# drdh/Homophily-MARL

Measured on AMD Instinct MI355X. Metric: agent_steps_per_sec, higher is better.
Workload: dtype fp32

## Files before the change

__graft_entry__.py:

```python
import os
import subprocess
import sys

ROOT = os.path.dirname(os.path.abspath(__file__))
if ROOT not in sys.path:
    sys.path.insert(0, ROOT)

CSRC = os.path.join(ROOT, "homophily_marl_amd", "csrc")
HIP_SOURCES = ["ssd_env.hip", "ssd_learner.hip", "ssd_policy.hip", "ssd_policy_mfma.hip", "ssd_gru_seq.hip", "ssd_bmm.hip", "ssd_abi.hip"]
HIP_LIB = os.path.join(ROOT, "homophily_marl_amd", "libssd_hip.so")
HIPCC_FLAGS = ["--offload-arch=gfx950", "-O3", "-std=c++17", "-fPIC", "-shared", "-ffp-contract=off",
               "-fno-fast-math", "-Wall", "-Wno-unused-function", "-mllvm", "-amdgpu-kernarg-preload-count=14"]


def _stale(target, sources):
    if not os.path.exists(target):
        return True
    t = os.path.getmtime(target)
    return any(os.path.getmtime(s) > t for s in sources)


def build(force=False):
    srcs = [os.path.join(CSRC, s) for s in HIP_SOURCES]
    hdrs = [os.path.join(CSRC, h) for h in os.listdir(CSRC) if h.endswith(".h")] + [os.path.join(ROOT, "include", "ssd_hip.h")]
    if force or _stale(HIP_LIB, srcs + hdrs + [os.path.abspath(__file__)]):
        from concurrent.futures import ThreadPoolExecutor
        hipcc = os.environ.get("HIPCC", "/opt/rocm/bin/hipcc")
        objdir = os.path.join(ROOT, "build", "obj")
        os.makedirs(objdir, exist_ok=True)
        flags = [f for f in HIPCC_FLAGS if f != "-shared"]
        jobs = []
        for src in srcs:
            obj = os.path.join(objdir, os.path.basename(src)[:-4] + ".o")
            if force or _stale(obj, [src] + hdrs + [os.path.abspath(__file__)]):
                jobs.append([hipcc] + flags + ["-c", src, "-o", obj])
        for cmd in jobs:
            print("[build]", " ".join(cmd), flush=True)
        with ThreadPoolExecutor(max_workers=min(len(jobs), os.cpu_count() or 1) or 1) as pool:
            rcs = list(pool.map(subprocess.call, jobs))
        if any(rcs):
            raise RuntimeError("hipcc failed (%s)" % rcs)
        objs = [os.path.join(objdir, os.path.basename(src)[:-4] + ".o") for src in srcs]
        cmd = [hipcc, "--offload-arch=gfx950", "-shared", "-fPIC", "-o", HIP_LIB] + objs
        print("[build]", " ".join(cmd), flush=True)
        subprocess.check_call(cmd)
    from oracle import oracle_py
    oracle_py.build(force=force)
    ref_mk = os.path.join(ROOT, "oracle", "build_ref.py")
    if os.path.isdir("/root/reference") and os.path.exists(ref_mk):
        subprocess.check_call([sys.executable, ref_mk])
    import homophily_marl_amd
    from homophily_marl_amd import abi
    abi.load_library()


def smoke():
    import numpy as np
    import torch
    from homophily_marl_amd import abi
    from homophily_marl_amd.envs.native import NativeEnv
    from oracle.oracle_py import OracleEnv

    assert torch.cuda.is_available(), "smoke() needs a GPU"
    kw = dict(map="default5", num_agents=5, n_env=64, view_size=7, episode_limit=100, rng_mode=abi.RNG_COUNTER, seed=7)
    dev = NativeEnv("cleanup", device=0, **kw)
    orc = OracleEnv("cleanup", **kw)
    dev.reset(); orc.reset()
    g = torch.Generator().manual_seed(0)
    for t in range(20):
        acts = torch.randint(0, 9, (64, 5), generator=g, dtype=torch.int32)
        o = dev.step_observe(acts.cuda())
        r = orc.step(acts.numpy())
        assert (o["reward"].cpu().numpy() == r["reward"]).all(), "reward mismatch at step %d" % t
    st, so = dev.export_state(), orc.export_state()
    assert (st["grid"].cpu().numpy() == so["grid"]).all() and (st["pos"].cpu().numpy() == so["pos"]).all()
    assert (o["obs"].cpu().numpy() == orc.observe()["obs"]).all()
    assert dev.poll_error() == 0
    print("smoke ok: 64 envs x 20 steps bit-exact vs oracle; obs", tuple(o["obs"].shape))
    from homophily_marl_amd.run import load_config, setup
    N2, T2 = 32, 12
    cfg = load_config("cleanup", overrides=dict(
        runner="hip_graph", batch_size_run=N2, batch_size=8, buffer_size=N2, buffer_cpu_only=False, store_state=False, obs_storage="code",
        env_args=dict(num_agents=5, map="default5", episode_limit=T2, seed=3), use_cuda=True, save_model=False, runner_stats=False,
        learner_log_interval=10 ** 12))
    torch.manual_seed(0)
    ctx = setup(cfg)
    batch = ctx.runner.run(test_mode=False)
    acts = batch["actions"].squeeze(-1).cpu().numpy().astype(np.int32)
    rew = batch["reward"].cpu().numpy()
    ctx.buffer.insert_episode_batch(batch)
    sample = ctx.buffer.sample(cfg["batch_size"])
    ctx.learner.train(sample[:, :sample.max_t_filled()], ctx.runner.t_env, 0)
    torch.cuda.synchronize()
    assert ctx.runner.env.native.poll_error() == 0
    orc2 = OracleEnv("cleanup", map="default5", num_agents=5, n_env=N2, view_size=7, episode_limit=T2, rng_mode=abi.RNG_COUNTER, seed=3)
    orc2.reset()
    for t in range(T2):
        assert (orc2.step(acts[:, t])["reward"] == rew[:, t]).all(), "stored episode does not replay on the oracle at step %d" % t
    assert all(torch.isfinite(p).all() for p in ctx.mac.parameters())
    print("smoke ok: rollout kernels + learner kernels, %d envs x %d steps stored episode replays on the oracle, one train step" % (N2, T2))


if __name__ == "__main__":
    build(force="--force" in sys.argv)
    if "--smoke" in sys.argv:
        smoke()
```

homophily_marl_amd/abi.py:

```python
import ctypes as C
import os

ABI_VERSION = 10
MAX_AGENTS = 10
MAX_CELLS = 1024
MAX_SITES = 256

ENV_CLEANUP, ENV_HARVEST = 0, 1
RNG_TAPE, RNG_COUNTER = 0, 1
OBS_F32, OBS_BF16, OBS_U8, OBS_CODE = 0, 1, 2, 3
COLOR_SIMPLIFIED, COLOR_FULL = 0, 1
CODE_CLASS, CODE_CHANNEL_MASK = 0, 1
INPUT_LAST_ACTION, INPUT_AGENT_ID, INPUT_REWARD, INPUT_INC_REWARD, INPUT_DISTANCE, INPUT_AGENT_POS = 1, 2, 4, 8, 16, 32
INPUT_OTHERS_LAST_ACTION = 64
INPUT_GATHER_ONEHOT = 0x100
PREV_RECORD_BYTES = 16
INPUT_EXPLICIT = 0x80000000
STREAM_UNIFORM, STREAM_MOVE, STREAM_WASTE, STREAM_SPAWN_ROT = 0, 1, 2, 3

SSD_OK, SSD_ERR_INVALID, SSD_ERR_DEVICE, SSD_ERR_NOMEM, SSD_ERR_UNSUPPORTED = 0, -1, -2, -3, -4
ERRBIT_F16_RANGE = 32
ERR_BAD_RENDER = 64

COPY_BLOCKS_MAX = 32
# ... 217 lines not shown
    return {
        prefix + "abi_version": (C.c_int, []),
        prefix + "last_error": (C.c_char_p, []),
        prefix + "create": (C.c_int, [P(SsdConfig), P(vp)]),
        prefix + "destroy": (C.c_int, [vp]),
        prefix + "reset": (C.c_int, [vp, vp, P(SsdTape), P(SsdStepOut)] + st),
        prefix + "step": (C.c_int, [vp, vp, P(SsdTape), P(SsdStepOut)] + st),
        prefix + "observe": (C.c_int, [vp, P(SsdObsOut)] + st),
        prefix + "export_state": (C.c_int, [vp, P(SsdState)] + st),
        prefix + "import_state": (C.c_int, [vp, P(SsdState)] + st),
        prefix + "get_info": (C.c_int, [vp, P(SsdInfo)]),
        prefix + "build_inputs": (C.c_int, [i32, i32, i32, i32, vp, vp, vp, vp, f32, vp, i32, i32] + st),
        prefix + "incentive_transfer": (C.c_int, [i32, i32, i32, vp, vp, f32, f32, f32, f32,
                                                  vp, vp, vp, vp, vp, vp] + st),
    }


CPU_SIGNATURES = _sigs("ssd_cpu_", False)

vp, i32, i64, u32, u64, f32, P = C.c_void_p, C.c_int32, C.c_int64, C.c_uint32, C.c_uint64, C.c_float, C.POINTER
HIP_SIGNATURES = {name: (C.c_int, args) for name, args in {
    "ssd_step_observe": [vp, vp, P(SsdTape), P(SsdStepOut), P(SsdObsOut), vp],
    "ssd_poll_error": [vp, P(i32)],
    "ssd_set_render": [vp, i32],
    "ssd_render": [vp, vp, i32, vp, vp, i64, vp],
    "ssd_unroll_other": [vp] * 6 + [f32] + [i32] * 4 + [vp] * 3,
    "ssd_column_sums": [vp, vp, i32, i32, i32, vp, vp],
    "ssd_dueling_q_fwd": [vp] * 3 + [i32] * 5 + [vp],
    "ssd_dueling_q_bwd": [vp] * 3 + [i32] * 5 + [vp],
    "ssd_gather_rows": [vp, i32, vp, i32, vp],
    "ssd_sample_ids": [u64, u32, i32, i32, vp, vp],
    "ssd_copy_blocks": [vp, i32, vp],
    "ssd_fill_blocks": [vp, i32, vp],
    "ssd_runner_stats": [vp, vp, vp, i32, i32, vp, vp],
    "ssd_behaviour_stats": [P(SsdBehaviourArgs), vp],
    "ssd_sample_windows": [u64, u32, i32, i32, i32, vp, vp, vp],
    "ssd_gather_windows": [vp, i32, vp, vp, i32, i32, i32, i32, vp],
    "ssd_priority_sample": [P(SsdPrioritySampleArgs), vp],
    "ssd_priority_update": [P(SsdPriorityUpdateArgs), vp],
    "ssd_rollout_priority": [P(SsdRolloutPriorityArgs), vp],
    "ssd_clip_adam_step": [P(SsdClipAdamArgs), vp],
    "ssd_td_sim_loss": [P(SsdTdLossArgs), i32, vp],
    "ssd_encoder": [vp, i32, i32, i32, i32, vp, vp, vp, vp, vp, i32, i32, i32, vp, i64, vp, vp],
    "ssd_conv_leaky": [vp, i32, i32, i32, vp, vp, vp, i32, i32, vp, i64, vp, vp],
    "ssd_store_step_launch": [P(SsdStoreStep), vp],
    "ssd_store_hidden": [P(SsdStoreHiddenArgs), vp],
    "ssd_gru_gates": [vp, vp, vp, i32, i32, vp],
    "ssd_gru_gates_fwd": [vp] * 5 + [i32, i32, vp],
    "ssd_gru_gates_bwd": [vp] * 7 + [i32, i32, vp],
    "ssd_dueling_pick": [vp, i32, i32, vp, vp, vp, u32, i32, i32, i32, vp, vp, u32, vp],
    "ssd_gru_seq_fwd": [vp] * 6 + [i32] * 3 + [vp],
    "ssd_gru_seq_bwd": [vp] * 9 + [i32] * 3 + [vp],
    "ssd_gru_seq_fwd_parts": [vp, i32, vp, vp, i32] + [vp] * 3 + [i32] * 3 + [vp],
    "ssd_gru_seq_bwd_parts": [vp] * 5 + [i32, vp, i32] + [vp] * 3 + [i32] * 4 + [vp],
    "ssd_gru_seq_fwd_h0": [vp, i32, vp, vp, i32, vp, i64, i64] + [vp] * 3 + [i32] * 3 + [vp],
    "ssd_gru_seq_bwd_h0": [vp] * 5 + [i32, vp, i32] + [vp] * 3 + [i32] * 4 + [vp],
    "ssd_bias_bmm_fwd": [vp] * 4 + [i32] * 4 + [vp],
    "ssd_bias_bmm_leaky_fwd": [vp] * 4 + [i32] * 4 + [vp],
    "ssd_bias_bmm_leaky_bwd": [vp] * 8 + [i32] * 4 + [vp],
    "ssd_bias_bmm_bwd": [vp] * 7 + [i32] * 4 + [vp],
    "ssd_bias_bmm2_fwd": [vp] * 5 + [i32] * 7 + [vp],
    "ssd_bias_bmm2_bwd_w": [vp] * 5 + [i32] * 7 + [vp],
    "ssd_bias_bmm_bwd_x": [vp] * 3 + [i32] * 4 + [i64, vp],
    "ssd_dueling_head_fwd": [vp] * 2 + [i32] * 5 + [vp],
    "ssd_dueling_head_bwd": [vp] * 3 + [i32] * 5 + [vp],
    "ssd_bmm_reserve_scratch": [vp],
    "ssd_set_learner_precision": [i32],
    "ssd_learner_precision": [],
    "ssd_conv_wgrad_partial_rows": [i32],
    "ssd_conv_wgrad_codes": [vp, vp, vp, i32, i32, vp],
    "ssd_build_inputs_width": [i32, i32, u32],
    "ssd_build_inputs_flags": [i32, i32, i32, i32, u32, vp, vp, vp, vp, f32, vp, i32, i32, vp],
    "ssd_policy_head_env": [P(SsdPolicyHead), vp],
    "ssd_policy_head_inc": [P(SsdPolicyHead), vp],
    "ssd_policy_head_plan": [i32] * 3 + [P(i32)] * 3,
    "ssd_policy_pack_head": [P(SsdPolicyHeadParams), i32, vp, vp],
    "ssd_policy_encode": [P(SsdPolicyEncodeArgs), vp],
    "ssd_policy_head_inc_encode": [P(SsdPolicyHead), P(SsdPolicyEncodeArgs), vp],
    "ssd_policy_pack_encoder_lut": [vp, vp, vp, i32, i32, vp, vp, vp],
    "ssd_policy_pack_encoder": [vp, vp, vp, i32, i32, vp, vp, vp],
    "ssd_numeric_status": [P(i32)],
}.items()}
HIP_SIGNATURES.update(_sigs("ssd_", True))


def onehot_rows(n_agents, n_actions, flags):
    return 1 + 2 * n_actions + (n_agents * n_actions if flags & INPUT_OTHERS_LAST_ACTION else 0)


def policy_image_bytes(precision):
    return (56 * precision + 8) * 1024


def policy_tail_piece(precision):
    return 56 * precision + 2 * precision


def policy_frag_piece(precision, F, term):
    if F < 8:
        c, ot = F & 1, F >> 1
    elif F < 56:
        G = (F - 8) % 24
        c, ot = (8 if F >= 32 else 2) + 2 * (G >> 3) + (G & 1), (G & 7) >> 1
    else:
        return 56 * precision + 2 * term + (F - 56)
    return 4 * precision * c + 4 * term + ot


def policy_head_plan(n_env, n_agents, fused_with_encoder=False):
    lib = load_library()
    a, b, c = C.c_int32(0), C.c_int32(0), C.c_int32(0)
    check(lib, lib.ssd_policy_head_plan(n_env, n_agents, int(fused_with_encoder), C.byref(a), C.byref(b), C.byref(c)))
    return a.value, b.value, c.value


def encode_edge_supported(V):
    return ENCODE_EDGE_MIN <= V <= ENCODE_EDGE_MAX and V % 2 == 1


def encode_band_rows(V):
    O = V - 2
    nb = 1 if O <= 13 else min(ENCODE_BANDS_MAX, (O + 9) // 10)
    return (O + nb - 1) // nb


def encode_bands(V):
    return (V - 2 + encode_band_rows(V) - 1) // encode_band_rows(V)


def encode_lut_ksteps(V):
    O, R, nb = V - 2, encode_band_rows(V), encode_bands(V)
    return (nb - 1) * ((R * O + 3) // 4) + ((O - (nb - 1) * R) * O + 3) // 4


def encode_frag_bytes(V, precision, layout=ENCODE_LAYOUT_TOEPLITZ):
    if layout == ENCODE_LAYOUT_LUT:
        return ENCODE_LUT_TABLE_BYTES, encode_lut_ksteps(V) * 2 * precision * 1024
    units = 29 * 2 * 3 if V == 31 else 13 * 3
    return precision * 9 * 1024, units * 2 * precision * 1024


def code_agent_stride(V):
    return (V * V + 15) & ~15


def behaviour_len(n, A):
    return 12 * n + n * A + 3 * n * n + 3


def behaviour_layout(n, A):
    blocks = (("reward_sum", (n,)), ("clean_sum", (n,)), ("clean_steps", (n,)), ("harvest_steps", (n,)), ("harvest_time", (n,)),
              ("action_count", (n, A)), ("inc_count", (n, n, 3)), ("recv_on_clean", (n,)), ("recv_on_reward", (n,)), ("role_count", (n, 4)),
              ("cleaners_hist", (n + 1,)), ("n_episodes", (1,)), ("n_steps", (1,)))
    out, off = {}, 0
    for name, shape in blocks:
        out[name] = (off, shape)
        size = 1
        for s in shape:
            size *= s
        off += size
    assert off == behaviour_len(n, A)
    return out


def behaviour_blocks(vec, n, A):
    import numpy as np
    vec = np.asarray(vec, dtype=np.float64).reshape(-1)
    assert vec.size == behaviour_len(n, A), (vec.size, n, A)
    return {k: vec[o:o + int(np.prod(s))].reshape(s).copy() for k, (o, s) in behaviour_layout(n, A).items()}


def behaviour_summary(vec, n, A):
    b = behaviour_blocks(vec, n, A)
    n_ep, n_steps = max(1.0, float(b["n_episodes"][0])), max(1.0, float(b["n_steps"][0]))
    inc, roles = b["inc_count"], b["role_count"].sum(axis=0)
    pairs = max(1, n * (n - 1)) * n_steps
    clean = b["clean_sum"]
    out = {"cleaners_per_env_mean": float((b["cleaners_hist"] * range(n + 1)).sum() / n_ep)}
    for k, name in enumerate(BEHAVIOUR_ROLES):
        out["role_%s_frac" % name] = float(roles[k] / (n * n_ep))
    out["inc_pos_rate"] = float(inc[..., 1].sum() / pairs)
    out["inc_neg_rate"] = float(inc[..., 2].sum() / pairs)
    out["rollout_incentives_to_cleanup_per"] = float(b["recv_on_clean"].sum() / (b["clean_steps"].sum() + 1e-6))
    out["rollout_incentives_to_harvest_per"] = float(b["recv_on_reward"].sum() / (b["reward_sum"].sum() + 1e-6))
    out["rollout_value_give_mean"] = float((inc[..., 1].sum() + inc[..., 2].sum()) / (n * n_steps))
    out["rollout_value_receive_mean"] = float((inc[..., 1].sum() - inc[..., 2].sum()) / (n * n_steps))
    out["harvest_time_mean"] = float(b["harvest_time"].sum() / max(1.0, b["harvest_steps"].sum()))
    out["clean_share_max"] = float(clean.max() / clean.sum()) if clean.sum() > 0 else 0.0
    return out


_PKG_DIR = os.path.dirname(os.path.abspath(__file__))
HIP_LIB_PATH = os.environ.get("SSD_HIP_LIB_PATH", os.path.join(_PKG_DIR, "libssd_hip.so"))
_lib = None


def bind(lib, signatures):
    missing = []
    for name, (res, args) in signatures.items():
        try:
            fn = getattr(lib, name)
        except AttributeError:
            missing.append(name)
            continue
        fn.restype = res
        fn.argtypes = args
    if missing:
        raise ImportError("native library is missing symbols: " + ", ".join(missing))
    return lib


def load_library():
    global _lib
    if _lib is None:
        import torch
        if not os.path.exists(HIP_LIB_PATH):
            raise ImportError(
                "%s not found: build it with `python -c 'import __graft_entry__ as g; g.build()'` "
                "(hipcc --offload-arch=gfx950).  There is no CPU fallback." % HIP_LIB_PATH)
        lib = C.CDLL(HIP_LIB_PATH)
        bind(lib, HIP_SIGNATURES)
        ver = lib.ssd_abi_version()
        if ver != ABI_VERSION:
            raise ImportError("libssd_hip.so ABI version %d != %d" % (ver, ABI_VERSION))
        _lib = lib
    return _lib


class SsdError(RuntimeError):
    pass


def check(lib, rc, err_fn="ssd_last_error"):
    if rc != 0:
        msg = getattr(lib, err_fn)()
        raise SsdError("ssd error %d: %s" % (rc, msg.decode() if msg else "?"))
```

homophily_marl_amd/controllers/homophily_controller.py:

```python
import numpy as np
import torch as th
import torch.nn as nn
import torch.nn.functional as F

from ..components.action_selectors import REGISTRY as action_REGISTRY
from ..modules.agents import REGISTRY as agent_REGISTRY
from .. import ops


class HomophilyMAC(nn.Module):
    def __init__(self, scheme, groups, args):
        super().__init__()
        self.n_agents = args.n_agents
        self.args = args
        self.shipped_flags = bool(args.obs_last_action and args.obs_agent_id and args.obs_reward and args.obs_inc_reward
                                  and args.obs_agent_pos and not getattr(args, "obs_others_last_action", False)
                                  and not getattr(args, "obs_distance", False))
        self.input_flags = None if getattr(args, "obs_others_last_action", False) else (
            1 * bool(args.obs_last_action) | 2 * bool(args.obs_agent_id) | 4 * bool(args.obs_reward) | 8 * bool(args.obs_inc_reward)
            | 16 * bool(getattr(args, "obs_distance", False)) | 32 * bool(args.obs_agent_pos))
        self.input_flags_all = ((self.input_flags if self.input_flags is not None else
                                 (1 * bool(args.obs_last_action) | 2 * bool(args.obs_agent_id) | 4 * bool(args.obs_reward)
                                  | 8 * bool(args.obs_inc_reward) | 16 * bool(getattr(args, "obs_distance", False)) | 32 * bool(args.obs_agent_pos)))
                                | 64 * bool(getattr(args, "obs_others_last_action", False)))
# ... 90 lines not shown
            ops.build_inputs_tail(tail, 0, last_actions, last_reward, last_actions_inc, pos, self.pos_scale, A, t0,
                                  flags=None if self.shipped_flags else self.input_flags_all)
            return th.cat([feat, tail], dim=1)
        dev = feat.device
        if t0:
            last_actions = th.full((B, n), -1, dtype=th.long, device=dev)
            last_reward = th.zeros(B, n, device=dev)
            last_actions_inc = th.zeros(B, n, n, dtype=th.long, device=dev)
        had = (last_actions >= 0).unsqueeze(-1).float()
        onehot = F.one_hot(last_actions.clamp(min=0), A).float() * had
        parts = [feat.reshape(B, n, F0)]
        if a.obs_last_action:
            parts.append(onehot)
        if a.obs_agent_id:
            parts.append(th.eye(n, device=dev).unsqueeze(0).expand(B, -1, -1))
        if a.obs_reward:
            parts.append(th.sign(last_reward.float()).unsqueeze(-1))
        if a.obs_inc_reward:
            m = last_actions_inc * self.inc_mask_actions.squeeze(-1).to(last_actions_inc.dtype)
            recv = (m == 1).sum(dim=1) - (m == 2).sum(dim=1)
            parts.append(th.sign(recv.float()).unsqueeze(-1))
        if getattr(a, "obs_others_last_action", False):
            parts.append(onehot.reshape(B, 1, n * A).expand(-1, n, -1))
        if getattr(a, "obs_distance", False):
            parts.append(1.0 - (pos.unsqueeze(2) - pos.unsqueeze(1)).norm(dim=-1) / self.pos_scale)
        if a.obs_agent_pos:
            parts.append(pos / self.pos_scale)
        return th.cat([x.reshape(B * n, -1).float() for x in parts], dim=1)

    def unroll(self, batch):
        shared = self.unroll_shared(batch)
        parts, wh, bh = self.unroll_pre(batch, shared)
        he, hi = ops.gru_sequence_parts(parts, batch.max_seq_length, batch.batch_size, wh, bh, h0=self.stored_h0(batch))
        return self.agent.unroll_post(he, hi, shared["other"])

    def stored_h0(self, batch):
        if not getattr(self.args, "train_stored_state", False):
            return None
        H = self.args.rnn_hidden_dim
        h = batch["hidden"][:, 0].detach()
        return [h[..., :H].transpose(0, 1), h[..., H:].transpose(0, 1)]

    def unroll_shared(self, batch):
        a = self.args
        B, T, n = batch.batch_size, batch.max_seq_length, self.n_agents
        obs = batch["obs"]
        codes = None
        if obs.dtype == th.uint8:
            if a.rgb_input and self.agent.encoder_kernel_shape and ops.encode_codes_supported(obs):
                codes = obs
            else:
                ops._leaving_kernels("encode_codes", obs, "no encoder kernel for %s windows" % (tuple(obs.shape[-2:]),))
                obs = self.expand_codes(obs)
        acts = batch["actions"].squeeze(-1)
        prev = lambda x, fill: th.cat([th.full_like(x[:, :1], fill), x[:, :-1]], dim=1)
        on_dev = batch["reward"].is_cuda
        kernel_tail = (self.shipped_flags or on_dev) and a.rgb_input and self.input_shape > a.obs_dim_net
        hist = None if (kernel_tail and on_dev) else (
            prev(acts, -1).reshape(B * T, n), prev(batch["reward"], 0).reshape(B * T, n),
            prev(batch["actions_inc"].squeeze(-1), 0).reshape(B * T, n, n), batch["agent_pos"].reshape(B * T, n, 2))
        sh = dict(obs=None if codes is not None else (obs.float() if a.rgb_input else obs), codes=codes, hist=hist, tail=None)
        if on_dev and acts.dtype == th.long:
            sh["onehot"] = None
            sh["other"], sh["act_tm"] = ops.unroll_other(acts, batch["agent_pos"], batch["agent_orientation"], batch["reward"], batch["clean_num"],
                                                         batch["apple_den"], self.pos_scale, a.n_actions)
        else:
            onehot = F.one_hot(acts, num_classes=a.n_actions)
            sh.update(onehot=onehot, act_tm=None,
                      other=self.agent.unroll_other(onehot, batch["agent_pos"] / self.pos_scale, batch["agent_orientation"], batch["reward"],
                                                    batch["clean_num"], batch["apple_den"], th.float32))
        if kernel_tail:
            tail = th.empty(B * T * n, self.input_shape - a.obs_dim_net, dtype=th.float32, device=batch["obs"].device)
            flags = None if self.shipped_flags else self.input_flags_all
            if hist is None:
                ops.build_inputs_tail(tail, 0, acts.reshape(B * T, n), batch["reward"].reshape(B * T, n),
                                      batch["actions_inc"].squeeze(-1).reshape(B * T, n, n), batch["agent_pos"].reshape(B * T, n, 2),
                                      self.pos_scale, a.n_actions, False, flags=flags, seq_len=T)
            else:
                ops.build_inputs_tail(tail, 0, hist[0], hist[1], hist[2], hist[3], self.pos_scale, a.n_actions, False, flags=flags)
            sh["tail"] = tail
        return sh

    def unroll_pre(self, batch, shared):
        a = self.args
        B, T, n = batch.batch_size, batch.max_seq_length, self.n_agents
        obs = shared["obs"]
        if shared.get("codes") is not None:
            feat = self.agent.rgb_preprocess_codes(shared["codes"].reshape(B * T * n, a.obs_dims[0], a.obs_dims[1]))
        elif a.rgb_input:
            feat = self.agent.rgb_preprocess(obs.reshape(B * T * n, 3, a.obs_dims[0], a.obs_dims[1]))
        else:
            feat = obs.reshape(B * T * n, -1)
        if shared["tail"] is not None:
            inputs = th.cat([feat, shared["tail"]], dim=1).reshape(B, T, n, -1)
        else:
            inputs = self.assemble_inputs(feat, *shared["hist"], False).reshape(B, T, n, -1)
        return self.agent.unroll_pre(inputs, shared["onehot"], act_tm=shared.get("act_tm"))

    def _build_inputs(self, batch, t):
        if self.args.rgb_input:
            feat = self.encode_obs(batch["obs"][:, t])
        else:
            feat = batch["obs"][:, t].reshape(batch.batch_size * self.n_agents, -1)
        if t == 0:
            return self.assemble_inputs(feat, None, None, None, batch["agent_pos"][:, t], True)
        return self.assemble_inputs(feat, batch["actions"][:, t - 1].squeeze(-1), batch["reward"][:, t - 1],
                                    batch["actions_inc"][:, t - 1].squeeze(-1), batch["agent_pos"][:, t], False)

    def _get_input_shape(self, scheme):
        a = self.args
        shape = a.obs_dim_net if a.rgb_input else scheme["obs"]["vshape"]
        if a.obs_last_action:
            shape += scheme["actions_onehot"]["vshape"][0]
        if a.obs_agent_id:
            shape += self.n_agents
        shape += int(bool(a.obs_reward)) + int(bool(a.obs_inc_reward))
        if getattr(a, "obs_others_last_action", False):
            shape += scheme["actions_onehot"]["vshape"][0] * self.n_agents
        if getattr(a, "obs_distance", False):
            shape += self.n_agents
        if a.obs_agent_pos:
            shape += 2
        return shape
```

homophily_marl_amd/csrc/ssd_abi.hip:

```cpp
#include <cmath>
#include <cstdio>
#include <cstring>
#include <new>
#include <vector>

#include "ssd_device.h"

using namespace ssd;

struct ssd_env {
    DevSpec hs;
    DevSpec* dspec;
    DevState st;
    int device;
    int n_spawn;
    uint32_t* beam_rec;
    uint8_t* render_lut;
    uint8_t host_lut[64];
};

static thread_local char g_err[512] = "";
static int fail(int code, const char* fmt, const char* a = "") {
    std::snprintf(g_err, sizeof g_err, fmt, a);
    return code;
}
#define HIP_TRY(expr)                                                                   \
    do {                                                                                \
        hipError_t e_ = (expr);                                                         \
        if (e_ != hipSuccess) return fail(SSD_ERR_DEVICE, #expr ": %s", hipGetErrorString(e_)); \
    } while (0)

static uint32_t magic(uint32_t d) { return d <= 1 ? 0xFFFFFFFFu : (uint32_t)(0x100000000ull / d) + 1u; }

extern "C" {

int ssd_abi_version(void) { return SSD_ABI_VERSION; }
const char* ssd_last_error(void) { return g_err; }

static uint32_t draw_threshold(double p) { return p >= 1.0 ? (1u << 24) : !(p > 0.0) ? 0u : (uint32_t)std::ceil(p * 16777216.0); }

int ssd_create(const ssd_config* cfg, ssd_env** out) {
    if (!cfg || !out || !cfg->ascii_map) return fail(SSD_ERR_INVALID, "null argument");
    if (cfg->n_agents < 1 || cfg->n_agents > SSD_MAX_AGENTS) return fail(SSD_ERR_INVALID, "n_agents out of range (1..10)");
    if (cfg->height < 3 || cfg->width < 3 || cfg->height > 255 || cfg->width > 255 || cfg->height * cfg->width > SSD_MAX_CELLS)
        return fail(SSD_ERR_INVALID, "map size out of range");
    if (cfg->n_env < 1) return fail(SSD_ERR_INVALID, "n_env must be >= 1");
    if (cfg->view_size < 0 || cfg->view_size > 31) return fail(SSD_ERR_INVALID, "view_size out of range (0..31)");
    {
        const long V = 2L * cfg->view_size + 1, pm = (cfg->height + 2L * cfg->view_size) * (cfg->width + 2L * cfg->view_size);
        const long per_wave = 2L * ((cfg->height * cfg->width + 15) & ~15) + pm + 16 + cfg->n_agents * 3L * V * V + 32 + 64 + (cfg->n_agents * SSD_CODE_AGENT_STRIDE(V) <= 2560 ? cfg->n_agents : 1) * SSD_CODE_AGENT_STRIDE(V) + 16;
        if (per_wave * 4 > 160 * 1024) return fail(SSD_ERR_INVALID, "map / view_size / n_agents exceed the LDS budget of one workgroup");
    }
    if (cfg->spawn_rotation > 3) return fail(SSD_ERR_INVALID, "spawn_rotation must be -1..3");
    if (cfg->env_kind != SSD_ENV_CLEANUP && cfg->env_kind != SSD_ENV_HARVEST) return fail(SSD_ERR_INVALID, "env_kind");
    if (cfg->rng_mode != SSD_RNG_TAPE && cfg->rng_mode != SSD_RNG_COUNTER) return fail(SSD_ERR_INVALID, "rng_mode");

    ssd_env* E = new (std::nothrow) ssd_env();
    if (!E) return fail(SSD_ERR_NOMEM, "host allocation failed");
    std::memset(E, 0, sizeof *E);
    DevSpec& S = E->hs;
    S.kind = cfg->env_kind; S.H = cfg->height; S.W = cfg->width; S.HW = S.H * S.W; S.GS = (S.HW + 15) & ~15;
    S.n = cfg->n_agents; S.N = cfg->n_env; S.v = cfg->view_size; S.V = 2 * S.v + 1; S.VV = S.V * S.V; S.VVp = (S.VV + 3) & ~3;
    S.Wp = S.W + 2 * S.v; S.PMS = ((S.H + 2 * S.v) * S.Wp + 15) & ~15;
    S.vshift = 0; while ((1 << S.vshift) < S.V) ++S.vshift;
    S.episode_limit = cfg->episode_limit; S.spawn_rotation = cfg->spawn_rotation < 0 ? -1 : cfg->spawn_rotation;
    S.obs_color = cfg->obs_color == SSD_COLOR_FULL ? SSD_COLOR_FULL : SSD_COLOR_SIMPLIFIED;
    S.rng_mode = cfg->rng_mode; S.n_actions = S.kind == SSD_ENV_CLEANUP ? 9 : 8;
    S.env_id_base = cfg->env_id_base; S.seed_lo = (uint32_t)cfg->seed; S.seed_hi = (uint32_t)(cfg->seed >> 32);
    S.magic_W = magic(S.W); S.magic_V = magic(S.V); S.magic_VV = magic(S.VV); S.magic_3VV = magic(3 * S.VV); S.magic_HW = magic(S.HW);
    S.thr_dep = cfg->threshold_depletion; S.thr_res = cfg->threshold_restoration;
    S.p_waste = cfg->waste_spawn_prob; S.p_apple = cfg->apple_respawn_prob;
    for (int i = 0; i < 4; ++i) { S.harvest_p[i] = cfg->harvest_spawn_prob[i]; S.harvest_thr[i] = draw_threshold(S.harvest_p[i]); }
    if ((long)S.n * 3 * S.VV >= 65536) { delete E; return fail(SSD_ERR_INVALID, "n_agents * 3 * V * V must stay below 65536"); }
    if ((long)lds_per_wave(S) * kWavesPerBlock > 160 * 1024) { delete E; return fail(SSD_ERR_INVALID, "k_env's LDS slices exceed the 160 KiB of a workgroup"); }
    if (code_gather_end(S, kCodeGroupMax) > lds_planes_bytes(S)) { delete E; return fail(SSD_ERR_INVALID, "class-code gather overruns its LDS planes"); }

    std::vector<int> spawn;
    for (int i = 0; i < S.HW; ++i) {
        const char ch = cfg->ascii_map[i];
        uint8_t code = C_EMPTY;
        bool overflow = false;
        if (ch == '@') code = C_WALL;
        else if (ch == 'P') spawn.push_back(i);
        else if (S.kind == SSD_ENV_CLEANUP) {
            if (ch == 'B') { if (S.n_apple < SSD_MAX_SITES) S.apple[S.n_apple++] = (uint16_t)i; else overflow = true; }
            else if (ch == 'H') { code = C_WASTE; if (S.n_waste < SSD_MAX_SITES) S.waste[S.n_waste++] = (uint16_t)i; else overflow = true; }
            else if (ch == 'R') code = C_RIVER;
            else if (ch == 'S') code = C_STREAM;
        } else if (ch == 'A') { code = C_APPLE; if (S.n_apple < SSD_MAX_SITES) S.apple[S.n_apple++] = (uint16_t)i; else overflow = true; }
// ... 680 lines not shown
                       (long)h0_row_stride);
    return launched();
}

int ssd_gru_seq_bwd(const float* dhs, const float* hs, const float* rzn, const float* ghn, const float* wh, float* d_gi, float* dgh,
                    float* d_wh, float* d_bh_part, int32_t T, int32_t G, int32_t B, void* stream) {
    if (int rc = gru_seq_bwd_check("ssd_gru_seq_bwd", 0, &dhs, hs, rzn, ghn, &wh, 1, &d_gi, 0, dgh, d_wh, d_bh_part, T, G, G, B)) return rc;
    launch_gru_seq_bwd(&dhs, hs, rzn, ghn, &wh, 1, &d_gi, 0, dgh, d_wh, d_bh_part, T, G, G, B, (hipStream_t)stream);
    return launched();
}
int ssd_gru_seq_bwd_parts(const float* const* dhs_parts, const float* hs, const float* rzn, const float* ghn, const float* const* wh_parts, int32_t n_wparts,
                          float* const* d_gi_parts, int32_t n_parts, float* dgh, float* d_wh, float* d_bh_part, int32_t T, int32_t G, int32_t G_grad, int32_t B,
                          void* stream) {
    if (int rc = gru_seq_bwd_check("ssd_gru_seq_bwd_parts", 1, dhs_parts, hs, rzn, ghn, wh_parts, n_wparts, d_gi_parts, n_parts, dgh, d_wh, d_bh_part, T, G, G_grad, B))
        return rc;
    launch_gru_seq_bwd(dhs_parts, hs, rzn, ghn, wh_parts, n_wparts, d_gi_parts, n_parts, dgh, d_wh, d_bh_part, T, G, G_grad, B, (hipStream_t)stream);
    return launched();
}
int ssd_gru_seq_bwd_h0(const float* const* dhs_parts, const float* hs, const float* rzn, const float* ghn, const float* const* wh_parts, int32_t n_wparts,
                       float* const* d_gi_parts, int32_t n_parts, float* dgh, float* d_wh, float* d_bh_part, int32_t T, int32_t G, int32_t G_grad, int32_t B,
                       void* stream) {
    if (int rc = gru_seq_bwd_check("ssd_gru_seq_bwd_h0", 0, dhs_parts, hs, rzn, ghn, wh_parts, n_wparts, d_gi_parts, n_parts, dgh, d_wh, d_bh_part, T, G, G_grad, B))
        return rc;
    launch_gru_seq_bwd(dhs_parts, hs, rzn, ghn, wh_parts, n_wparts, d_gi_parts, n_parts, dgh, d_wh, d_bh_part, T, G, G_grad, B, (hipStream_t)stream, true);
    return launched();
}

int ssd_bias_bmm_fwd(const float* x, const float* w, const float* b, float* y, int32_t n, int32_t rows, int32_t in, int32_t out, void* stream) {
    if (!x || !w || !b || !y || n < 1 || rows < 1 || in < 1 || out < 1) return fail(SSD_ERR_INVALID, "bad argument");
    if (launch_bias_bmm_fwd(x, w, b, y, n, rows, in, out, (hipStream_t)stream)) return fail(SSD_ERR_UNSUPPORTED, "ssd_bias_bmm_fwd: a weight / operand set of 2^30 elements or more");
    return launched();
}
int ssd_bias_bmm_leaky_fwd(const float* x, const float* w, const float* b, float* y, int32_t n, int32_t rows, int32_t in, int32_t out, void* stream) {
    if (!x || !w || !b || !y || n < 1 || rows < 1 || in < 1 || out < 1) return fail(SSD_ERR_INVALID, "bad argument");
    if (launch_bias_bmm_fwd(x, w, b, y, n, rows, in, out, (hipStream_t)stream, 1)) return fail(SSD_ERR_UNSUPPORTED, "ssd_bias_bmm_leaky_fwd: a weight / operand set of 2^30 elements or more");
    return launched();
}
int ssd_bias_bmm_leaky_bwd(const float* g, const float* y, const float* x, const float* w, float* dx, float* dw, float* db, const float* slope_of,
                           int32_t n, int32_t rows, int32_t in, int32_t out, void* stream) {
    if (!g || !y || n < 1 || rows < 1 || in < 1 || out < 1) return fail(SSD_ERR_INVALID, "bad argument");
    if ((dx && !w) || ((dw || db) && !x) || (slope_of && !dx)) return fail(SSD_ERR_INVALID, "dx needs w, dw / db need x, slope_of needs dx");
    if (launch_bias_bmm_bwd(g, x, w, dx, dw, db, slope_of, n, rows, in, out, (hipStream_t)stream, 0, 0, y)) return fail(SSD_ERR_UNSUPPORTED, "ssd_bias_bmm_leaky_bwd: an operand set of 2^30 elements or more");
    return launched();
}
int ssd_bias_bmm_bwd(const float* g, const float* x, const float* w, float* dx, float* dw, float* db, const float* slope_of, int32_t n,
                     int32_t rows, int32_t in, int32_t out, void* stream) {
    if (!g || n < 1 || rows < 1 || in < 1 || out < 1) return fail(SSD_ERR_INVALID, "bad argument");
    if ((dx && !w) || ((dw || db) && !x) || (slope_of && !dx)) return fail(SSD_ERR_INVALID, "dx needs w, dw / db need x, slope_of needs dx");
    if (launch_bias_bmm_bwd(g, x, w, dx, dw, db, slope_of, n, rows, in, out, (hipStream_t)stream)) return fail(SSD_ERR_UNSUPPORTED, "ssd_bias_bmm_bwd: an operand set of 2^30 elements or more");
    return launched();
}

int ssd_dueling_head_fwd(const float* y, float* q, int32_t n, int32_t T, int32_t B, int32_t inner, int32_t K, void* stream) {
    if (!y || !q || n < 1 || T < 1 || B < 1 || inner < 1 || K < 1 || K > 15) return fail(SSD_ERR_INVALID, "bad argument");
    launch_dueling_q(y, y + K, q, nullptr, nullptr, nullptr, n, T, B, inner, K, (hipStream_t)stream, K + 1, 1, nullptr);
    return launched();
}
int ssd_dueling_head_bwd(const float* dq, float* dy, float* gs, int32_t n, int32_t T, int32_t B, int32_t inner, int32_t K, void* stream) {
    if (!dq || !dy || n < 1 || T < 1 || B < 1 || inner < 1 || K < 1 || K > 15) return fail(SSD_ERR_INVALID, "bad argument");
    launch_dueling_q(nullptr, nullptr, nullptr, dq, dy, dy + K, n, T, B, inner, K, (hipStream_t)stream, K + 1, 1, gs);
    return launched();
}
int ssd_bias_bmm2_fwd(const float* x1, const float* x2, const float* w, const float* b, float* y, int32_t n, int32_t rows, int32_t in1, int32_t in2,
                      int32_t out, int32_t x1_div, int32_t x2_shared, void* stream) {
    if (!x1 || !x2 || !w || !b || !y || n < 1 || rows < 1 || in1 < 1 || in2 < 1 || out < 1) return fail(SSD_ERR_INVALID, "bad argument");
    const int rc = launch_bias_bmm2_fwd(x1, x2, w, b, y, n, rows, in1, in2, out, x1_div, x2_shared, (hipStream_t)stream);
    if (rc == -3) return fail(SSD_ERR_INVALID, "ssd_bias_bmm2_fwd: in1 a multiple of 16, rows a multiple of x1_div >= 1");
    if (rc) return fail(SSD_ERR_UNSUPPORTED, "ssd_bias_bmm2_fwd: a weight / operand set of 2^30 elements or more");
    return launched();
}
int ssd_bias_bmm2_bwd_w(const float* g, const float* x1, const float* x2, float* dw, float* db, int32_t n, int32_t rows, int32_t in1, int32_t in2,
                        int32_t out, int32_t x1_div, int32_t x2_shared, void* stream) {
    if (!g || !x1 || !x2 || (!dw && !db) || n < 1 || rows < 1 || in1 < 1 || in2 < 1 || out < 1) return fail(SSD_ERR_INVALID, "bad argument");
    const int rc = launch_bias_bmm_bwd(g, x1, nullptr, nullptr, dw, db, nullptr, n, rows, in1 + in2, out, (hipStream_t)stream, 0, 0, nullptr, x2, in1, x1_div,
                                       x2_shared, 0);
    if (rc == -3) return fail(SSD_ERR_INVALID, "ssd_bias_bmm2_bwd_w: in1 a multiple of 16, rows a multiple of x1_div >= 1");
    if (rc) return fail(SSD_ERR_UNSUPPORTED, "ssd_bias_bmm2_bwd_w: an operand set of 2^30 elements or more");
    return launched();
}
int ssd_bias_bmm_bwd_x(const float* g, const float* w, float* dx, int32_t n, int32_t rows, int32_t in, int32_t out, int64_t w_set, void* stream) {
    if (!g || !w || !dx || n < 1 || rows < 1 || in < 1 || out < 1 || w_set < (int64_t)in * out) return fail(SSD_ERR_INVALID, "bad argument");
    if (launch_bias_bmm_bwd(g, nullptr, w, dx, nullptr, nullptr, nullptr, n, rows, in, out, (hipStream_t)stream, 0, 0, nullptr, nullptr, 0, 1, 0, (long)w_set))
        return fail(SSD_ERR_UNSUPPORTED, "ssd_bias_bmm_bwd_x: an operand set of 2^30 elements or more");
    return launched();
}
int ssd_bmm_reserve_scratch(void* stream) {
    if (!bmm_scratch((hipStream_t)stream)) return fail(SSD_ERR_DEVICE, "ssd_bmm_reserve_scratch: allocation failed (inside a stream capture?)");
    return SSD_OK;
}
int ssd_set_learner_precision(int32_t precision) {
    if (precision != 1 && precision != 2) return fail(SSD_ERR_INVALID, "ssd_set_learner_precision: 1 (bf16) or 2 (f32)");
    set_learner_precision(precision);
    return SSD_OK;
}
int ssd_learner_precision(void) { return learner_precision(); }
int ssd_conv_wgrad_partial_rows(int32_t rows) { return rows < 1 ? 0 : conv_wgrad_partial_rows(rows); }
static bool encode_edge_ok(int V) { return V >= SSD_ENCODE_EDGE_MIN && V <= SSD_ENCODE_EDGE_MAX && (V & 1); }
#define SSD_EDGE_MSG ": view_edge must be odd, 3 .. 63 (view_size 1 .. 31)"

int ssd_conv_wgrad_codes(const uint8_t* codes, const float* d_conv, float* partial, int32_t rows, int32_t view_edge, void* stream) {
    if (!codes || !d_conv || !partial || rows < 1) return fail(SSD_ERR_INVALID, "bad argument");
    if (!encode_edge_ok(view_edge)) return fail(SSD_ERR_UNSUPPORTED, "ssd_conv_wgrad_codes" SSD_EDGE_MSG);
    if (launch_conv_wgrad(codes, d_conv, partial, rows, view_edge, (hipStream_t)stream)) return fail(SSD_ERR_UNSUPPORTED, "ssd_conv_wgrad_codes" SSD_EDGE_MSG);
    return launched();
}

static int check_encode(const ssd_policy_encode_args* a) {
    if (!a || !a->codes || !a->conv_frags || !a->lin_frags || !a->conv_b || !a->lin_b || a->rows < 1 || a->n_agents < 1 || a->rows % a->n_agents)
        return fail(SSD_ERR_INVALID, "bad argument");
    if (!encode_edge_ok(a->view_edge)) return fail(SSD_ERR_UNSUPPORTED, "ssd_policy_encode" SSD_EDGE_MSG "; use ssd_conv_leaky + GEMM");
    const bool shipped = a->view_edge == 15 || a->view_edge == 31;
    if (!shipped && a->layout != SSD_ENCODE_LAYOUT_LUT)
        return fail(SSD_ERR_UNSUPPORTED, "ssd_policy_encode: the Toeplitz layout is instantiated for 15 x 15 / 31 x 31 windows; other edges take SSD_ENCODE_LAYOUT_LUT");
    if (a->precision != 0 && a->precision != 1 && a->precision != 2) return fail(SSD_ERR_INVALID, "precision must be 1 (bf16) or 2 (f32-equivalent)");
    if (a->alphabet != SSD_CODE_CLASS && a->alphabet != SSD_CODE_CHANNEL_MASK) return fail(SSD_ERR_INVALID, "alphabet");
    if (a->layout != SSD_ENCODE_LAYOUT_TOEPLITZ && a->layout != SSD_ENCODE_LAYOUT_LUT) return fail(SSD_ERR_INVALID, "layout");
    if (a->act && shipped && a->layout != SSD_ENCODE_LAYOUT_TOEPLITZ)
        return fail(SSD_ERR_INVALID, "the activation output (training forward) takes the Toeplitz images at 15 x 15 / 31 x 31");
    const int bands = SSD_ENCODE_BANDS(a->view_edge);
    if (bands == 1 ? (!a->out || a->part || a->out_stride < 32) : (!a->part || a->out)) return fail(SSD_ERR_INVALID, "one band writes `out`, several bands write `part`");
    if ((reinterpret_cast<uintptr_t>(a->conv_frags) | reinterpret_cast<uintptr_t>(a->lin_frags) | reinterpret_cast<uintptr_t>(a->part)) & 15)
        return fail(SSD_ERR_INVALID, "conv_frags / lin_frags / part must be 16-byte aligned");
    const long VV = (long)a->view_edge * a->view_edge;
    if (a->agent_stride < VV || a->env_stride < (long)a->n_agents * a->agent_stride || a->slot_stride < 0 || (a->slot_stride && !a->slot_t))
        return fail(SSD_ERR_INVALID, "env_stride / slot_stride / agent_stride / slot_t");
    if (a->code_bytes < (long)(a->rows / a->n_agents - 1) * a->env_stride + (long)(a->n_agents - 1) * a->agent_stride + VV)
        return fail(SSD_ERR_INVALID, "code_bytes does not cover the rows");
    if (a->slot_t_copy && (!a->slot_t || a->slot_t_copy == a->slot_t)) return fail(SSD_ERR_INVALID, "slot_t_copy needs a distinct slot_t");
    if (a->slot_add < 0 || (a->slot_add && !a->slot_t)) return fail(SSD_ERR_INVALID, "slot_add needs slot_t");
    return SSD_OK;
}

int ssd_policy_encode(const ssd_policy_encode_args* a, void* stream) {
    if (const int bad = check_encode(a)) return bad;
    const int rc = launch_policy_encode(a, (hipStream_t)stream);
    if (rc) return fail(SSD_ERR_DEVICE, "hipFuncSetAttribute(max dynamic LDS) failed");
    return launched();
}

int ssd_policy_pack_encoder_lut(const float* conv_w, const float* conv_b, const float* lin_w, int32_t view_edge, int32_t precision, void* table,
                                void* lin_frags, void* stream) {
    if (!conv_w || !conv_b || !lin_w || !table || !lin_frags) return fail(SSD_ERR_INVALID, "null argument");
    if (precision != 1 && precision != 2) return fail(SSD_ERR_INVALID, "precision must be 1 or 2");
    if ((reinterpret_cast<uintptr_t>(table) | reinterpret_cast<uintptr_t>(lin_frags)) & 15) return fail(SSD_ERR_INVALID, "images must be 16-byte aligned");
    if (!encode_edge_ok(view_edge)) return fail(SSD_ERR_UNSUPPORTED, "ssd_policy_pack_encoder_lut" SSD_EDGE_MSG);
    if (launch_pack_encoder_lut(conv_w, conv_b, lin_w, view_edge, precision, table, lin_frags, (hipStream_t)stream))
        return fail(SSD_ERR_UNSUPPORTED, "ssd_policy_pack_encoder_lut" SSD_EDGE_MSG);
    return launched();
}

int ssd_policy_pack_encoder(const float* conv_w, const float* conv_b, const float* lin_w, int32_t view_edge, int32_t precision, void* conv_frags,
                            void* lin_frags, void* stream) {
    if (!conv_w || !conv_b || !lin_w || !conv_frags || !lin_frags) return fail(SSD_ERR_INVALID, "null argument");
    if (precision != 1 && precision != 2) return fail(SSD_ERR_INVALID, "precision must be 1 or 2");
    if ((reinterpret_cast<uintptr_t>(conv_frags) | reinterpret_cast<uintptr_t>(lin_frags)) & 15) return fail(SSD_ERR_INVALID, "fragment images must be 16-byte aligned");
    if (launch_pack_encoder(conv_w, conv_b, lin_w, view_edge, precision, conv_frags, lin_frags, (hipStream_t)stream))
        return fail(SSD_ERR_UNSUPPORTED, "ssd_policy_pack_encoder: view_edge must be 15 or 31");
    return launched();
}

int ssd_policy_pack_head(const ssd_policy_head_params* p, int32_t precision, void* image, void* stream) {
    if (!p || !image || !p->fc1_w || !p->fc1_b || !p->fc2_w || !p->fc2_b || !p->fc2_v_w || !p->fc2_v_b) return fail(SSD_ERR_INVALID, "null argument");
    for (int g = 0; g < 3; ++g) if (!p->w_i[g] || !p->w_h[g] || !p->b_i[g] || !p->b_h[g]) return fail(SSD_ERR_INVALID, "null GRU parameter");
    if (precision != 1 && precision != 2) return fail(SSD_ERR_INVALID, "precision must be 1 or 2");
    if (p->input_flags & SSD_INPUT_GATHER_ONEHOT) {
        const uint32_t fl = p->input_flags;
// ... 154 lines not shown
```

homophily_marl_amd/csrc/ssd_bmm.hip:

```cpp
#include <hip/hip_runtime.h>
#include <mutex>
#include <stdint.h>
#include "../../include/ssd_hip.h"

namespace ssd {

using f32x4 = __attribute__((ext_vector_type(4))) float;
typedef float f32x4_u __attribute__((ext_vector_type(4), aligned(4)));

struct BmmK {
    const float *x, *w, *b, *g;
    float *y, *dx, *dw, *db;
    const float* slope_of;
    int n, R, I, O;
    long x_set, g_set;
    const float* act_y;
    int leaky;
    const float* x2; int I1, x1_div; long x2_set;
    uint32_t x1_magic;
    long w_set;
    float* part;
    int row_chunks;
};
constexpr int BMM_PART = 272;

__device__ __forceinline__ float ld32(const float* base, uint32_t idx) {
    return *reinterpret_cast<const float*>(reinterpret_cast<const uint8_t*>(base) + (size_t)(idx * 4u));
}
__device__ __forceinline__ f32x4 mfma4(float a, float b, f32x4 c) { return __builtin_amdgcn_mfma_f32_16x16x4f32(a, b, c, 0, 0, 0); }
using bf8 = __attribute__((ext_vector_type(8))) __bf16;
__device__ __forceinline__ f32x4 mfma32b(const float (&a)[8], const float (&b)[8], f32x4 c) {
    bf8 x, y;
#pragma unroll
    for (int j = 0; j < 8; ++j) { x[j] = (__bf16)a[j]; y[j] = (__bf16)b[j]; }
    return __builtin_amdgcn_mfma_f32_16x16x32_bf16(x, y, c, 0, 0, 0);
}
static int g_learner_precision = 2;
int learner_precision() { return g_learner_precision; }
void set_learner_precision(int p) { g_learner_precision = p == 1 ? 1 : 2; }

__device__ __forceinline__ f32x4 load4(const float* p, int k0, int len) {
    if (k0 + 4 <= len) return *reinterpret_cast<const f32x4_u*>(p + k0);
    f32x4 v = {0.f, 0.f, 0.f, 0.f};
#pragma unroll
    for (int r = 0; r < 4; ++r)
        if (k0 + r < len) v[r] = p[k0 + r];
    return v;
}

constexpr int BMM_TPW = 3;
template <bool XV, bool BF = false>
__global__ __launch_bounds__(256) void k_bias_bmm_fwd(BmmK a) {
    const int lane = threadIdx.x & 63, wave = __builtin_amdgcn_readfirstlane(threadIdx.x >> 6);
    const int m = lane & 15, q = lane >> 4;
    const int R = a.R, I = a.I, O = a.O;
    const int otiles = (O + 15) >> 4, groups = (otiles + BMM_TPW - 1) / BMM_TPW, rtiles = (R + 15) >> 4;
    const int unit = blockIdx.x * 4 + wave;
    if (unit >= rtiles * groups) return;
    const int g = blockIdx.y, row0 = (unit / groups) * 16, t0 = (unit % groups) * BMM_TPW;
    const int rowc = row0 + m < R ? row0 + m : R - 1;
    const bool two = a.x2 != nullptr;
    const int I1 = two ? a.I1 : I;
    const float* xs = a.x + (two ? (size_t)g * (size_t)(R / a.x1_div) * I1 : (size_t)g * R * I);
    const uint32_t xrow = two ? (uint32_t)(rowc / a.x1_div) * (uint32_t)I1 : (uint32_t)rowc * (uint32_t)I;
    const float* x2s = two ? a.x2 + (size_t)g * a.x2_set : a.x;
    const uint32_t x2row = (uint32_t)rowc * (uint32_t)(I - I1);
    const float* wg = a.w + (size_t)g * (a.w_set ? a.w_set : (long)I * O);
    f32x4 acc[BMM_TPW];
#pragma unroll
    for (int t = 0; t < BMM_TPW; ++t) {
        const int o = 16 * (t0 + t) + m;
        const float bv = (t0 + t < otiles && o < O) ? a.b[(size_t)g * O + o] : 0.f;
        acc[t] = f32x4{bv, bv, bv, bv};
    }
    const int chunks = (I + 15) >> 4;
    int oc[BMM_TPW]; bool on[BMM_TPW];
#pragma unroll
    for (int t = 0; t < BMM_TPW; ++t) {
        const int o = 16 * (t0 + t) + m;
        on[t] = t0 + t < otiles && o < O; oc[t] = on[t] ? o : 0;
    }
    struct Chunk { float x[4]; float w[BMM_TPW][4]; };
    auto fetch = [&](int c, Chunk& d) {
        const int k0 = 16 * c + 4 * q;
        if constexpr (XV) {
            const int kc = k0 < I ? k0 : I - 4;
            const bool second = 16 * c >= I1;
            const float* base = second ? x2s : xs;
            const uint32_t off = second ? x2row + (uint32_t)(kc - I1) : xrow + (uint32_t)kc;
            const f32x4 v = *reinterpret_cast<const f32x4_u*>(reinterpret_cast<const uint8_t*>(base) + (size_t)(off * 4u));
#pragma unroll
            for (int r = 0; r < 4; ++r) d.x[r] = v[r];
        }
#pragma unroll
        for (int r = 0; r < 4; ++r) {
            const int k = k0 + r < I ? k0 + r : I - 1;
            if constexpr (!XV) {
                const bool sec = k >= I1;
                d.x[r] = ld32(sec ? x2s : xs, sec ? x2row + (uint32_t)(k - I1) : xrow + (uint32_t)k);
            }
#pragma unroll
            for (int t = 0; t < BMM_TPW; ++t) d.w[t][r] = ld32(wg, (uint32_t)k * (uint32_t)O + (uint32_t)oc[t]);
        }
    };
    auto use = [&](int c, const Chunk& d) {
        const int k0 = 16 * c + 4 * q;
#pragma unroll
        for (int r = 0; r < 4; ++r) {
            const bool kon = k0 + r < I;
            const float xv = kon ? d.x[r] : 0.f;
#pragma unroll
            for (int t = 0; t < BMM_TPW; ++t)
                if (t0 + t < otiles) acc[t] = mfma4(xv, (kon && on[t]) ? d.w[t][r] : 0.f, acc[t]);
        }
    };
    auto use_pair = [&](int c, const Chunk& d0, const Chunk& d1, bool two) {
        const int k0 = 16 * c + 4 * q;
        float xv[8];
#pragma unroll
        for (int r = 0; r < 4; ++r) { xv[r] = k0 + r < I ? d0.x[r] : 0.f; xv[4 + r] = (two && k0 + 16 + r < I) ? d1.x[r] : 0.f; }
#pragma unroll
        for (int t = 0; t < BMM_TPW; ++t) {
            if (t0 + t >= otiles) continue;
            float wv[8];
#pragma unroll
            for (int r = 0; r < 4; ++r) { wv[r] = (k0 + r < I && on[t]) ? d0.w[t][r] : 0.f; wv[4 + r] = (two && k0 + 16 + r < I && on[t]) ? d1.w[t][r] : 0.f; }
            acc[t] = mfma32b(xv, wv, acc[t]);
        }
    };
    Chunk ca, cb;
    fetch(0, ca);
    for (int c = 0; c < chunks; c += 2) {
        if (c + 1 < chunks) fetch(c + 1, cb);
        if constexpr (BF) {
            Chunk cur = ca;
            if (c + 2 < chunks) fetch(c + 2, ca);
            use_pair(c, cur, cb, c + 1 < chunks);
        } else {
            use(c, ca);
            if (c + 1 < chunks) {
                if (c + 2 < chunks) fetch(c + 2, ca);
                use(c + 1, cb);
            }
        }
    }
#pragma unroll
    for (int t = 0; t < BMM_TPW; ++t) {
        const int o = 16 * (t0 + t) + m;
        if (t0 + t >= otiles || o >= O) continue;
#pragma unroll
        for (int r = 0; r < 4; ++r) {
            const int row = row0 + 4 * q + r;
            const float v = acc[t][r];
            if (row < R) a.y[((size_t)g * R + row) * O + o] = (a.leaky && !(v > 0.f)) ? 0.01f * v : v;
        }
    }
}

__device__ __forceinline__ int gridDim_tiles(const BmmK& a) { return ((a.I + 15) >> 4) * ((a.O + 15) >> 4); }
__global__ __launch_bounds__(64) void k_bmm_dw_reduce(BmmK a) {
    const int lane = threadIdx.x, m = lane & 15, q = lane >> 4, tile = blockIdx.x, g = blockIdx.y, C = a.row_chunks;
    const int otiles = (a.O + 15) >> 4, it = tile / otiles, ot = tile - it * otiles, o = 16 * ot + m;
    const float* P = a.part + ((size_t)((size_t)g * gridDim.x + tile) * C) * BMM_PART;
    f32x4 sum = *reinterpret_cast<const f32x4*>(P + 4 * lane);
    float sb = q == 0 ? P[256 + m] : 0.f;
    for (int c = 1; c < C; ++c) {
        sum += *reinterpret_cast<const f32x4*>(P + (size_t)c * BMM_PART + 4 * lane);
        if (q == 0) sb += P[(size_t)c * BMM_PART + 256 + m];
    }
    if (o >= a.O) return;
    if (a.dw) {
#pragma unroll
        for (int r = 0; r < 4; ++r) {
            const int ii = 16 * it + 4 * q + r;
            if (ii < a.I) a.dw[((size_t)g * a.I + ii) * a.O + o] = sum[r];
        }
    }
    if (a.db && it == 0 && q == 0) a.db[(size_t)g * a.O + o] = sb;
}
constexpr int BMM_BWD_WAVES = 16;
template <bool OV, bool ACT, bool BF = false>
__global__ __launch_bounds__(BMM_BWD_WAVES * 64) void k_bias_bmm_bwd(BmmK a, int dw_blocks) {
    __shared__ f32x4 red[BMM_BWD_WAVES][64];
    __shared__ float redb[BMM_BWD_WAVES][16];
    const int lane = threadIdx.x & 63, wave = __builtin_amdgcn_readfirstlane(threadIdx.x >> 6);
    const int m = lane & 15, q = lane >> 4;
    const int g = blockIdx.y;
    const int R = a.R, I = a.I, O = a.O;
    const int itiles = (I + 15) >> 4, otiles = (O + 15) >> 4;
    const float* gg = a.g + (size_t)g * a.g_set;
    if ((int)blockIdx.x >= dw_blocks) {
        const int unit = (blockIdx.x - dw_blocks) * BMM_BWD_WAVES + wave, rtiles = (R + 15) >> 4;
        if (unit >= rtiles * itiles) return;
        const int row0 = (unit / itiles) * 16, i = 16 * (unit % itiles) + m;
        const int rowc = row0 + m < R ? row0 + m : R - 1;
        const float* ws = a.w + (size_t)g * (a.w_set ? a.w_set : (long)I * O);
        const uint32_t grow = (uint32_t)rowc * (uint32_t)O, wrow = (uint32_t)(i < I ? i : I - 1) * (uint32_t)O;
        f32x4 acc = {0.f, 0.f, 0.f, 0.f};
        const int chunks = (O + 15) >> 4;
        struct Pair { f32x4 g, w, y; };
        const float* yy = ACT ? a.act_y + (size_t)g * a.g_set : nullptr;
        auto fetch = [&](int c, Pair& d) {
            const int k0 = 16 * c + 4 * q;
            if constexpr (OV) {
                const uint32_t kb = (uint32_t)(k0 < O ? k0 : O - 4);
                d.g = *reinterpret_cast<const f32x4_u*>(reinterpret_cast<const uint8_t*>(gg) + (size_t)((grow + kb) * 4u));
                d.w = *reinterpret_cast<const f32x4_u*>(reinterpret_cast<const uint8_t*>(ws) + (size_t)((wrow + kb) * 4u));
                if constexpr (ACT) d.y = *reinterpret_cast<const f32x4_u*>(reinterpret_cast<const uint8_t*>(yy) + (size_t)((grow + kb) * 4u));
            } else {
#pragma unroll
                for (int r = 0; r < 4; ++r) {
                    const uint32_t k = (uint32_t)(k0 + r < O ? k0 + r : O - 1);
                    d.g[r] = ld32(gg, grow + k); d.w[r] = ld32(ws, wrow + k);
                    if constexpr (ACT) d.y[r] = ld32(yy, grow + k);
                }
            }
        };
        auto use = [&](int c, const Pair& d) {
            const int k0 = 16 * c + 4 * q;
#pragma unroll
            for (int r = 0; r < 4; ++r) {
                const bool on = k0 + r < O;
                float gv = on ? d.g[r] : 0.f;
                if constexpr (ACT) gv = d.y[r] > 0.f ? gv : 0.01f * gv;
                acc = mfma4(gv, on ? d.w[r] : 0.f, acc);
            }
        };
        auto use_pair = [&](int c, const Pair& d0, const Pair& d1, bool two) {
            const int k0 = 16 * c + 4 * q;
            float gv[8], wv[8];
#pragma unroll
            for (int r = 0; r < 4; ++r) {
                const bool on0 = k0 + r < O, on1 = two && k0 + 16 + r < O;
                float g0 = on0 ? d0.g[r] : 0.f, g1 = on1 ? d1.g[r] : 0.f;
                if constexpr (ACT) { g0 = d0.y[r] > 0.f ? g0 : 0.01f * g0; g1 = (on1 && !(d1.y[r] > 0.f)) ? 0.01f * g1 : g1; }
                gv[r] = g0; gv[4 + r] = g1; wv[r] = on0 ? d0.w[r] : 0.f; wv[4 + r] = on1 ? d1.w[r] : 0.f;
            }
// ... 91 lines not shown
        if (C > 1) {
            float* P = a.part + ((size_t)((size_t)g * gridDim_tiles(a) + tile) * C + chunk) * BMM_PART;
            *reinterpret_cast<f32x4*>(P + 4 * lane) = sum;
            if (q == 0) {
                float sb = redb[0][m];
#pragma unroll
                for (int v = 1; v < BMM_BWD_WAVES; ++v) sb += redb[v][m];
                P[256 + m] = sb;
            }
            return;
        }
        if (a.dw && oon) {
#pragma unroll
            for (int r = 0; r < 4; ++r) {
                const int ii = 16 * it + 4 * q + r;
                if (ii < I) a.dw[((size_t)g * I + ii) * O + o] = sum[r];
            }
        }
        if (a.db && it == 0 && q == 0 && oon) {
            float sb = redb[0][m];
#pragma unroll
            for (int v = 1; v < BMM_BWD_WAVES; ++v) sb += redb[v][m];
            a.db[(size_t)g * O + o] = sb;
        }
    }
}

constexpr size_t BMM_SCRATCH_BYTES = 1 << 20;
constexpr int BMM_SCRATCH_SLOTS = 64;
float* bmm_scratch(hipStream_t stream) {
    struct Slot { hipStream_t stream; float* buf; };
    static Slot slots[64][BMM_SCRATCH_SLOTS] = {};
    static int used[64] = {};
    static std::mutex mu;
    int dev = 0;
    if (hipGetDevice(&dev) != hipSuccess || dev < 0 || dev >= 64) return nullptr;
    std::lock_guard<std::mutex> lock(mu);
    for (int i = 0; i < used[dev]; ++i)
        if (slots[dev][i].stream == stream) return slots[dev][i].buf;
    if (used[dev] == BMM_SCRATCH_SLOTS) return nullptr;
    float* p = nullptr;
    if (hipMalloc((void**)&p, BMM_SCRATCH_BYTES) != hipSuccess) { (void)hipGetLastError(); return nullptr; }
    slots[dev][used[dev]++] = Slot{stream, p};
    return p;
}

int launch_bias_bmm_fwd(const float* x, const float* w, const float* b, float* y, int n, int R, int I, int O, hipStream_t s, int leaky) {
    BmmK k = {};
    k.x = x; k.w = w; k.b = b; k.y = y; k.n = n; k.R = R; k.I = I; k.O = O; k.leaky = leaky;
    const int otiles = (O + 15) / 16, units = ((R + 15) / 16) * ((otiles + BMM_TPW - 1) / BMM_TPW);
    if ((long)I * O >= (1L << 30) || (long)R * I >= (1L << 30)) return -2;
    const dim3 grid((units + 3) / 4, n);
    if (g_learner_precision == 1) {
        if ((I & 3) == 0) hipLaunchKernelGGL((k_bias_bmm_fwd<true, true>), grid, dim3(256), 0, s, k);
        else hipLaunchKernelGGL((k_bias_bmm_fwd<false, true>), grid, dim3(256), 0, s, k);
    } else {
        if ((I & 3) == 0) hipLaunchKernelGGL((k_bias_bmm_fwd<true, false>), grid, dim3(256), 0, s, k);
        else hipLaunchKernelGGL((k_bias_bmm_fwd<false, false>), grid, dim3(256), 0, s, k);
    }
    return 0;
}

int launch_bias_bmm2_fwd(const float* x1, const float* x2, const float* w, const float* b, float* y, int n, int R, int I1, int I2, int O, int x1_div,
                         int x2_shared, hipStream_t s) {
    BmmK k = {};
    const int I = I1 + I2;
    k.x = x1; k.x2 = x2; k.I1 = I1; k.x1_div = x1_div; k.x2_set = x2_shared ? 0 : (long)R * I2;
    k.w = w; k.b = b; k.y = y; k.n = n; k.R = R; k.I = I; k.O = O;
    if ((I1 & 15) || x1_div < 1 || R % x1_div) return -3;
    if ((long)I * O >= (1L << 30) || (long)R * I >= (1L << 30)) return -2;
    const int otiles = (O + 15) / 16, units = ((R + 15) / 16) * ((otiles + BMM_TPW - 1) / BMM_TPW);
    const dim3 grid((units + 3) / 4, n);
    const bool xv = (I2 & 3) == 0;
    if (g_learner_precision == 1) {
        if (xv) hipLaunchKernelGGL((k_bias_bmm_fwd<true, true>), grid, dim3(256), 0, s, k);
        else hipLaunchKernelGGL((k_bias_bmm_fwd<false, true>), grid, dim3(256), 0, s, k);
    } else {
        if (xv) hipLaunchKernelGGL((k_bias_bmm_fwd<true, false>), grid, dim3(256), 0, s, k);
        else hipLaunchKernelGGL((k_bias_bmm_fwd<false, false>), grid, dim3(256), 0, s, k);
    }
    return 0;
}

int launch_bias_bmm_bwd(const float* g, const float* x, const float* w, float* dx, float* dw, float* db, const float* slope_of, int n, int R,
                        int I, int O, hipStream_t s, long x_set, long g_set, const float* act_y, const float* x2, int I1, int x1_div, int x2_shared,
                        long w_set) {
    BmmK k = {};
    k.act_y = act_y;
    if ((long)R * I >= (1L << 30) || (long)R * O >= (1L << 30) || (long)I * O >= (1L << 30)) return -2;
    if (x2) {
        if (dx || (I1 & 15) || x1_div < 1 || R % x1_div) return -3;
        k.x2 = x2; k.I1 = I1; k.x1_div = x1_div; k.x2_set = x2_shared ? 0 : (long)R * (I - I1);
        k.x1_magic = x1_div == 1 ? 0u : (uint32_t)(((1ull << 32) + (uint64_t)x1_div - 1) / (uint64_t)x1_div);
        if (R >= (1 << 28) || (uint64_t)R * (uint64_t)x1_div > (1ull << 32)) return -2;
    }
    k.w_set = w_set;
    k.g = g; k.x = x; k.w = w; k.dx = dx; k.dw = dw; k.db = db; k.slope_of = slope_of; k.n = n; k.R = R; k.I = I; k.O = O;
    k.x_set = x_set ? x_set : (long)R * I; k.g_set = g_set ? g_set : (long)R * O;
    const int dxb = dx ? (((R + 15) / 16) * ((I + 15) / 16) + BMM_BWD_WAVES - 1) / BMM_BWD_WAVES : 0;
    int dwb = (dw || db) ? ((I + 15) / 16) * ((O + 15) / 16) : 0;
    if (dxb + dwb == 0) return 0;
    k.row_chunks = 1;
    const int tiles = dwb;
    if (dwb && (R + 3) / 4 >= 64 * BMM_BWD_WAVES && dwb * n <= 128) {
        int c = 256 / (dwb * n);
        if (c > 8) c = 8;
        float* part = bmm_scratch(s);
        if (c > 1 && part && (size_t)n * dwb * c * BMM_PART * sizeof(float) <= BMM_SCRATCH_BYTES) { k.row_chunks = c; k.part = part; dwb *= c; }
    }
    const dim3 grid(dwb + dxb, n), block(BMM_BWD_WAVES * 64);
    const bool ov = (O & 3) == 0, bf = g_learner_precision == 1;
#define SSD_BWD(OV_, ACT_, BF_) hipLaunchKernelGGL((k_bias_bmm_bwd<OV_, ACT_, BF_>), grid, block, 0, s, k, dwb)
    if (act_y) {
        if (ov) { if (bf) SSD_BWD(true, true, true); else SSD_BWD(true, true, false); }
        else { if (bf) SSD_BWD(false, true, true); else SSD_BWD(false, true, false); }
    } else {
        if (ov) { if (bf) SSD_BWD(true, false, true); else SSD_BWD(true, false, false); }
        else { if (bf) SSD_BWD(false, false, true); else SSD_BWD(false, false, false); }
    }
#undef SSD_BWD
    if (k.row_chunks > 1) hipLaunchKernelGGL(k_bmm_dw_reduce, dim3(tiles, n), dim3(64), 0, s, k);
    return 0;
}


constexpr int CW_ROWS = 4, CW_OUT = 6 * 27 + 6;
template <int CTRL, int ROW_MASK>
__device__ __forceinline__ float dpp_add(float v) {
    return v + __builtin_bit_cast(float, __builtin_amdgcn_update_dpp(0, __builtin_bit_cast(int, v), CTRL, ROW_MASK, 0xF, false));
}
__device__ __forceinline__ float wave_sum_to_lane63(float v) {
    v = dpp_add<0xB1, 0xF>(v);
    v = dpp_add<0x4E, 0xF>(v);
    v = dpp_add<0x124, 0xF>(v);
    v = dpp_add<0x128, 0xF>(v);
    v = dpp_add<0x142, 0xA>(v);
    v = dpp_add<0x143, 0xC>(v);
    return v;
}
template <int V>
__global__ __launch_bounds__(256) void k_conv_wgrad(const uint8_t* __restrict__ codes, const float* __restrict__ d_conv, float* __restrict__ partial, int R) {
    constexpr int O = V - 2, P = O * O, VV = V * V, VVP = (VV + 15) & ~15;
    __shared__ uint8_t win[4][VVP];
    const int lane = threadIdx.x & 63, wave = __builtin_amdgcn_readfirstlane(threadIdx.x >> 6);
    const int wg = blockIdx.x * 4 + wave;
    float acc[6][27], accb[6];
#pragma unroll
    for (int oc = 0; oc < 6; ++oc) {
        accb[oc] = 0.f;
#pragma unroll
        for (int k = 0; k < 27; ++k) acc[oc][k] = 0.f;
    }
    constexpr int PASSES = (P + 63) / 64;
    const int row_begin = wg * CW_ROWS, rows_here = row_begin >= R ? 0 : (R - row_begin < CW_ROWS ? R - row_begin : CW_ROWS);
    const int items = rows_here * PASSES;
    auto fetch = [&](int it, float (&v)[6]) {
        const int row = row_begin + it / PASSES, p = (it % PASSES) * 64 + lane;
        const float* dr = d_conv + (size_t)row * 6 * P;
#pragma unroll
        for (int oc = 0; oc < 6; ++oc) v[oc] = p < P ? dr[oc * P + p] : 0.f;
    };
    float cur[6], nxt[6];
    if (items > 0) fetch(0, nxt);
    for (int it = 0; it < items; ++it) {
#pragma unroll
        for (int oc = 0; oc < 6; ++oc) cur[oc] = nxt[oc];
// ... 123 lines not shown
```

homophily_marl_amd/csrc/ssd_device.h:

```cpp
#pragma once
#include <hip/hip_runtime.h>
#include <stdint.h>

#include "../../include/ssd_hip.h"

namespace ssd {

constexpr int kWave = 64;
#ifndef SSD_WAVES_PER_BLOCK
#define SSD_WAVES_PER_BLOCK 4
#endif
constexpr int kWavesPerBlock = SSD_WAVES_PER_BLOCK;
constexpr int kBlock = kWave * kWavesPerBlock;

enum : int { C_EMPTY = 0, C_WALL = 1, C_APPLE = 2, C_WASTE = 3, C_RIVER = 4, C_STREAM = 5 };
enum : int { O_LEFT = 0, O_RIGHT = 1, O_UP = 2, O_DOWN = 3 };
enum : int { MODE_RESET = 0, MODE_STEP = 1, MODE_STEP_OBS = 2, MODE_OBS = 3 };

struct DevHead {
    int32_t kind, H, W, HW, GS;
    int32_t n, N, V, v, VV, VVp;
    int32_t Wp, PMS;
    int32_t vshift;
    int32_t episode_limit, spawn_rotation, obs_color, rng_mode, n_actions;
// ... 30 lines not shown
    uint8_t* grid;
    uint2* agents;
    EnvHdr* hdr;
    int32_t* err;
    unsigned long long* stamps;
};

struct DevTape {
    const uint8_t* move_order;
    const double* uniforms;
    int32_t ustride;
    const uint8_t* waste_order;
    const uint8_t* spawn_rot;
    const uint8_t* spawn_order;
};

struct DevStepOut {
    float *reward, *clean_num, *apple_den;
    uint8_t* terminated;
    float *collective, *equality;
    int32_t* n_draws;
};

struct DevObsOut {
    void* obs;
    int32_t fmt;
    float *state, *pos, *orient;
    long env_stride, slot_stride;
    int32_t t_slots;
    uint8_t* code;
    int32_t code_agent_stride;
    unsigned long long* stamps;
};

enum : int { ERR_BAD_ACTION = 1, ERR_BAD_TAPE = 2, ERR_KEYERROR = 4, ERR_TAPE_OVERRUN = 8, ERR_SLOT_OVERRUN = 16, ERR_F16_RANGE = 32, ERR_BAD_RENDER = 64 };
int32_t* numeric_err_word();
constexpr float F16_MAX = 65504.f;

__host__ __device__ inline int lds_planes_bytes(const DevHead& s) { return ((s.n * 3 * s.VV + 16) + 15) & ~15; }
__host__ __device__ inline int code_dump_byte(int delta, int n, int VV) { return delta + n * VV; }
__host__ __device__ inline int code_gather_end(const DevHead& s, int ag) {
    return code_dump_byte(15, s.n, s.VV) + ((ag < s.n ? ag : s.n) - 1) * s.VV + 1;
}
constexpr int kCodeGroupMax = 5;
__host__ __device__ inline bool lds_code_all(const DevHead& s) { return s.n * SSD_CODE_AGENT_STRIDE(s.V) <= 2560; }
__host__ __device__ inline int lds_code_bytes(const DevHead& s) { return (lds_code_all(s) ? s.n : 1) * SSD_CODE_AGENT_STRIDE(s.V) + 16; }
#if defined(SSD_STAMPS) && SSD_STAMPS == 2
constexpr int kStampLds = 256;
#else
constexpr int kStampLds = 0;
#endif
__host__ __device__ inline int lds_per_wave(const DevHead& s) {
    int obs = s.PMS + lds_planes_bytes(s);
    if (obs < 512) obs = 512;
    return ((2 * s.GS + obs + 64 + lds_code_bytes(s) + 255) & ~255) + kStampLds;
}

void launch_env(int mode, const DevSpec* spec, const DevSpec& host_spec, DevState st, const int32_t* actions,
                const uint8_t* env_mask, DevTape tape, DevStepOut so, DevObsOut oo, hipStream_t stream, uint32_t* beam_rec = nullptr);
void launch_beam_clear(uint32_t* beam_rec, const uint8_t* env_mask, int n_env, int n_agents, hipStream_t stream);
void launch_render(const DevSpec* spec, const DevSpec& hs, DevState st, const uint32_t* beam_rec, const uint8_t* lut, const int32_t* env_ids,
                   int n_sel, uint8_t* frames, const int32_t* slot, long long slot_stride, hipStream_t stream);

void launch_export(const DevSpec* spec, const DevSpec& hs, DevState st, ssd_state dst, hipStream_t stream);
void launch_import(const DevSpec* spec, const DevSpec& hs, DevState st, ssd_state src, hipStream_t stream);

void launch_build_inputs(int32_t batch, int32_t n, int32_t A, int32_t t0, const int64_t* last_actions,
                         const float* last_reward, const int64_t* last_actions_inc, const float* pos, float pos_scale,
                         float* out, int32_t out_stride, int32_t out_offset, hipStream_t stream);
struct BuildInputsLayout { int o_act, o_id, o_r, o_i, o_oth, o_dist, o_pos, width; };
BuildInputsLayout build_inputs_layout(int n, int A, uint32_t input_flags);
void launch_build_inputs_flags(int32_t batch, int32_t n, int32_t A, int32_t t0, uint32_t input_flags, const int64_t* last_actions,
                               const float* last_reward, const int64_t* last_actions_inc, const float* pos, float pos_scale,
                               float* out, int32_t out_stride, int32_t out_offset, hipStream_t stream);
void launch_incentive_transfer(int32_t B, int32_t T, int32_t n, const int64_t* a_inc, const float* rewards,
                               float effect_ratio, float cost_ratio, float incentive, float seq_len, float* give,
                               float* recv_pos, float* recv_neg, float* recv_zero, float* r_env, float* r_inc,
                               hipStream_t stream);

void launch_column_sums(const float* x, float* out, int G, int R, int C, float* workspace, hipStream_t stream);
void launch_copy_blocks(const ssd_block_copy* blocks, int count, hipStream_t stream);
void launch_clip_adam(const ssd_clip_adam_args* a, hipStream_t stream);
void launch_dueling_q(const float* a, const float* v, float* q, const float* dq, float* da, float* dv, int n, int T, int B, int inner, int K, hipStream_t stream,
                      int ld = 0, int merged = 0, float* gs = nullptr);
void launch_gather_rows(const ssd_row_gather* fields, int count, const int64_t* ids, int n_ids, hipStream_t stream);
void launch_td_sim_loss(const ssd_td_loss_args* a, int mode, hipStream_t stream);
constexpr long long kDefaultLdsLimit = 64 * 1024;
constexpr int kEncoderRowsPerWave = 1, kEncoderRowsPerBlock = 4 * kEncoderRowsPerWave;
constexpr long long encoder_lds_bytes(long long V) { return kEncoderRowsPerBlock * (3 * V * V + 4) * (long long)sizeof(float); }
constexpr long long conv_leaky_lds_bytes(long long V) { return (3 * V * V + 6 * 27 + 6) * (long long)sizeof(float); }
void launch_encoder(const float* obs, int rows, int V, const float* cw, const float* cb, const float* lw, const float* lb, float* out,
                    int out_stride, int n_agents, int agent_major, float* store, long store_env_stride, const int64_t* store_t,
                    hipStream_t s);
void launch_conv_leaky(const float* obs, int rows, int V, const float* cw, const float* cb, float* out, int n_agents, int agent_major,
                       float* store, long store_env_stride, const int64_t* store_t, hipStream_t s);
void launch_store_step(const ssd_store_step* a, hipStream_t s);
void launch_store_hidden(const ssd_store_hidden_args* a, hipStream_t s);
void launch_gru_gates(const float* gi, const float* gh, float* h, int R, int H, hipStream_t s);
void launch_gru_fwd_train(const float* gi, const float* gh, const float* h, float* h_new, float* rzn, int R, int H, hipStream_t s);
void launch_gru_bwd(const float* dh, const float* rzn, const float* gh, const float* h, float* d_gi, float* d_gh, float* dh_prev, int R,
                    int H, hipStream_t s);
int launch_policy_encode(const ssd_policy_encode_args* p, hipStream_t s);
int launch_pack_encoder_lut(const float* cw, const float* cb, const float* lw, int V, int prec, void* table, void* lin_frags, hipStream_t s);
int launch_pack_encoder(const float* cw, const float* cb, const float* lw, int V, int prec, void* conv_frags, void* lin_frags, hipStream_t s);
void launch_pack_head(const ssd_policy_head_params* p, int prec, void* image, hipStream_t s);
void launch_gru_seq_fwd(const float* const* gi_parts, int n_parts, const float* const* wh_parts, const float* const* bh_parts, int n_wparts, float* hs,
                        float* rzn, float* ghn, int T, int G, int B, hipStream_t s, const float* const* h0_parts = nullptr, long h0_set_stride = 0,
                        long h0_row_stride = 0);
void launch_gru_seq_bwd(const float* const* dhs_parts, const float* hs, const float* rzn, const float* ghn, const float* const* wh_parts, int n_wparts,
                        float* const* d_gi_parts, int n_parts, float* dgh, float* d_wh, float* d_bh_part, int T, int G, int Gn, int B, hipStream_t s,
                        bool h0 = false);
int launch_policy_head(const ssd_policy_head* p, int inc, hipStream_t s);
void policy_head_plan(int n_env, int n_agents, int mode, int* wg_per_agent, int* waves_out, int* tiles_per_wave);
int launch_policy_inc_encode(const ssd_policy_head* ph, const ssd_policy_encode_args* pe, hipStream_t s);
int launch_policy_inc_encode_gather(const ssd_policy_head* ph, const ssd_policy_encode_args* pe, hipStream_t s);
int conv_wgrad_partial_rows(int R);
int launch_conv_wgrad(const uint8_t* codes, const float* d_conv, float* partial, int R, int V, hipStream_t s);
void launch_unroll_other(const int64_t* actions, const float* pos, const float* orient, const float* reward, const float* clean, const float* den,
                         float pos_scale, int B, int T, int n, int A, float* other, float* act_tm, hipStream_t stream);
float* bmm_scratch(hipStream_t stream);
int learner_precision();
void set_learner_precision(int p);
void launch_fill_blocks(const ssd_block_fill* blocks, int count, hipStream_t stream);
void launch_runner_stats(const float* coll, const float* eq, const float* ret, int n_env, int n_ret, double* acc, hipStream_t stream);
void launch_behaviour_stats(const ssd_behaviour_args* a, hipStream_t stream);
void launch_sample_draw(uint64_t seed, uint32_t call, int population, int count, int n_starts, int64_t* ids, int64_t* t0, hipStream_t stream);
void launch_gather_windows(const ssd_window_field* fields, int count, const int64_t* ids, const int64_t* t0, int n_ids, int src_slots,
                           int win_slots, int burn_in, hipStream_t stream);
void launch_priority_sample(const ssd_priority_sample_args* a, hipStream_t stream);
void launch_priority_update(const ssd_priority_update_args* a, hipStream_t stream);
void launch_rollout_priority(const ssd_rollout_priority_args* a, hipStream_t stream);
int launch_bias_bmm_fwd(const float* x, const float* w, const float* b, float* y, int n, int R, int I, int O, hipStream_t s, int leaky = 0);
int launch_bias_bmm_bwd(const float* g, const float* x, const float* w, float* dx, float* dw, float* db, const float* slope_of, int n, int R,
                        int I, int O, hipStream_t s, long x_set = 0, long g_set = 0, const float* act_y = nullptr, const float* x2 = nullptr, int I1 = 0,
                        int x1_div = 1, int x2_shared = 0, long w_set = 0);
int launch_bias_bmm2_fwd(const float* x1, const float* x2, const float* w, const float* b, float* y, int n, int R, int I1, int I2, int O, int x1_div,
                         int x2_shared, hipStream_t s);
#ifdef SSD_STAMPS
void set_policy_stamps(unsigned long long* buf);
#endif
void launch_dueling_pick(const float* av, int R, int A, const uint8_t* avail, const float* eps, const int64_t* step, uint32_t seed,
                         int n_agents, int B, int pairs, int64_t* actions, float* q_out, uint32_t env_id_base, hipStream_t s);

}
```

homophily_marl_amd/csrc/ssd_learner.hip:

```cpp
#include "ssd_device.h"

namespace ssd {

__global__ void k_build_inputs(int32_t rows, int32_t n, int32_t A, int32_t t0, const int64_t* __restrict__ last_actions,
                               const float* __restrict__ last_reward, const int64_t* __restrict__ last_actions_inc,
                               const float* __restrict__ pos, float pos_scale, float* __restrict__ out,
                               int32_t out_stride, int32_t out_offset) {
    const int width = A + n + 4;
    const size_t total = (size_t)rows * width;
    for (size_t idx = (size_t)blockIdx.x * blockDim.x + threadIdx.x; idx < total; idx += (size_t)gridDim.x * blockDim.x) {
        const int row = (int)(idx / width), k = (int)(idx - (size_t)row * width);
        const int b = row / n, i = row - b * n;
        const int agent_major = t0 & 2;
        const int hist_T = t0 >> 8;
        const int t_zero = (t0 & 1) || (hist_T && b % hist_T == 0);
        const size_t pb = hist_T ? (size_t)b - 1 : (size_t)b, prow = pb * n + i;
        float v;
        if (k < A) v = (!t_zero && last_actions[prow] == k) ? 1.f : 0.f;
        else if (k < A + n) v = (k - A == i) ? 1.f : 0.f;
        else if (k == A + n) {
            const float r = t_zero ? 0.f : last_reward[prow];
            v = (float)((r > 0.f) - (r < 0.f));
        } else if (k == A + n + 1) {
            int recv = 0;
// ... 500 lines not shown
__global__ __launch_bounds__(64 * BEH_WAVES) void k_behaviour_partials(const int64_t* __restrict__ actions, const int64_t* __restrict__ actions_inc,
                                                                       const float* __restrict__ reward, const float* __restrict__ clean,
                                                                       int n_env, int T, int n, int A, long long* __restrict__ ws) {
    __shared__ long long cnt[BEH_LEN_MAX];
    const int len = SSD_BEHAVIOUR_LEN(n, A);
    for (int k = threadIdx.x; k < len; k += 64 * BEH_WAVES) cnt[k] = 0;
    __syncthreads();
    const int lane = threadIdx.x & 63, wave = threadIdx.x >> 6;
    const int tpw = 64 / n, nn = n * n;
    const int tl = lane / n, j = lane - tl * n;
    const bool active = tl < tpw;
    const int o_act = 5 * n, o_inc = o_act + n * A, o_rc = o_inc + 3 * nn, o_role = o_rc + 2 * n, o_hist = o_role + 4 * n, o_ep = o_hist + n + 1;
    long long s_r = 0, s_c = 0, s_cl = 0, s_hv = 0, s_ht = 0, s_rc = 0, s_rr = 0, envs = 0;
    const size_t row = (size_t)(T + 1) * n;
    for (long b = (long)blockIdx.x * BEH_WAVES + wave; b < n_env; b += (long)gridDim.x * BEH_WAVES) {
        const int64_t* a_e = actions + (size_t)b * row;
        const int64_t* ai_e = actions_inc + (size_t)b * row * n;
        const float* r_e = reward + (size_t)b * row;
        const float* c_e = clean + (size_t)b * row;
        int C = 0, Hh = 0;
        for (int t0 = 0; t0 < T; t0 += tpw) {
            const int t = t0 + tl;
            const bool valid = active && t < T;
            const int tc = valid ? t : 0, m = tc * n + j;
            long long v[SSD_MAX_AGENTS];
#pragma unroll
            for (int i = 0; i < SSD_MAX_AGENTS; ++i) v[i] = ai_e[tc * nn + (i < n ? i : j) * n + j];
            const long long a = a_e[m];
            const int r = valid ? beh_round(r_e[m]) : 0, c = valid ? beh_round(c_e[m]) : 0;
            int rv = 0;
#pragma unroll
            for (int i = 0; i < SSD_MAX_AGENTS; ++i) {
                const bool ok = valid && i < n && i != j;
                if (ok && (unsigned long long)v[i] < 3ull) beh_add(cnt, o_inc + (i * n + j) * 3 + (int)v[i], 1);
                rv += (ok && v[i] == 1) - (ok && v[i] == 2);
            }
            if (valid && (unsigned long long)a < (unsigned long long)A) beh_add(cnt, o_act + j * A + (int)a, 1);
            const int cl = c > 0, hv = r > 0;
            s_r += r; s_c += c; s_cl += cl; s_hv += hv; s_ht += hv ? t : 0;
            s_rc += cl ? rv : 0; s_rr += (long long)r * rv;
            C += cl; Hh += hv;
        }
        int Cs = 0, Hs = 0;
        for (int k = 0; k < tpw; ++k) {
            const int src = (lane + k * n) & 63;
            Cs += __shfl(C, src); Hs += __shfl(Hh, src);
        }
        const bool agent = lane < n, cleaner = agent && Cs > Hs;
        if (agent) beh_add(cnt, o_role + lane * 4 + ((Cs == 0 && Hs == 0) ? 0 : Cs > Hs ? 1 : Hs > Cs ? 2 : 3), 1);
        const int n_cleaners = __popcll(__ballot(cleaner));
        if (lane == 0) beh_add(cnt, o_hist + n_cleaners, 1);
        envs += 1;
    }
    if (active) {
        beh_add(cnt, j, s_r); beh_add(cnt, n + j, s_c); beh_add(cnt, 2 * n + j, s_cl); beh_add(cnt, 3 * n + j, s_hv); beh_add(cnt, 4 * n + j, s_ht);
        beh_add(cnt, o_rc + j, s_rc); beh_add(cnt, o_rc + n + j, s_rr);
    }
    if (lane == 0) { beh_add(cnt, o_ep, envs); beh_add(cnt, o_ep + 1, envs * T); }
    __syncthreads();
    for (int k = threadIdx.x; k < len; k += 64 * BEH_WAVES) ws[(size_t)blockIdx.x * len + k] = cnt[k];
}

__global__ __launch_bounds__(256) void k_behaviour_finish(const long long* __restrict__ ws, int groups, int len, double* __restrict__ acc) {
    for (int k = threadIdx.x; k < len; k += 256) {
        long long s = 0;
        for (int g = 0; g < groups; ++g) s += ws[(size_t)g * len + k];
        acc[k] += (double)s;
    }
}

void launch_behaviour_stats(const ssd_behaviour_args* a, hipStream_t stream) {
    int groups = a->n_env / BEH_WAVES + (a->n_env % BEH_WAVES ? 1 : 0);
    if (groups > SSD_BEHAVIOUR_MAX_GROUPS) groups = SSD_BEHAVIOUR_MAX_GROUPS;
    long long* ws = reinterpret_cast<long long*>(a->workspace);
    hipLaunchKernelGGL(k_behaviour_partials, dim3(groups), dim3(64 * BEH_WAVES), 0, stream, a->actions, a->actions_inc, a->reward, a->clean_num,
                       a->n_env, a->t_slots - 1, a->n_agents, a->n_actions, ws);
    hipLaunchKernelGGL(k_behaviour_finish, dim3(1), dim3(256), 0, stream, ws, groups, SSD_BEHAVIOUR_LEN(a->n_agents, a->n_actions), a->acc);
}

static int grid_for(size_t total);
template <bool BWD>
__global__ __launch_bounds__(256) void k_dueling_q(const float* __restrict__ a, const float* __restrict__ v, float* __restrict__ q,
                                                   const float* __restrict__ dq, float* __restrict__ da, float* __restrict__ dv, int n, int T, int B,
                                                   int inner, int K, int ld, int merged, float* __restrict__ gs) {
    const long rows = (long)T * B * inner, total = rows * n;
    const int vld = merged ? ld : 1;
    for (long idx = (long)blockIdx.x * 256 + threadIdx.x; idx < total; idx += (long)gridDim.x * 256) {
        const int i = (int)(idx / rows);
        const long r = idx - (long)i * rows;
        const long tb = r / inner;
        const int j = (int)(r - tb * inner), t = (int)(tb / B), b = (int)(tb - (long)t * B);
        const size_t qo = ((((size_t)b * T + t) * n + i) * inner + j) * K, ao = ((size_t)i * rows + r) * ld;
        float x[16], sum = 0.f;
        for (int k = 0; k < K; ++k) { x[k] = BWD ? dq[qo + k] : a[ao + k]; sum += x[k]; }
        if (BWD) {
            const float mean = sum / (float)K;
            for (int k = 0; k < K; ++k) da[ao + k] = x[k] - mean;
            dv[((size_t)i * rows + r) * vld] = sum;
            if (gs && j == 0) {
                float g[17];
                for (int k = 0; k <= K; ++k) g[k] = 0.f;
                for (int jj = 0; jj < inner; ++jj) {
                    const size_t qj = qo + (size_t)jj * K;
                    float y[16], s2 = 0.f;
                    for (int k = 0; k < K; ++k) { y[k] = dq[qj + k]; s2 += y[k]; }
                    const float m2 = s2 / (float)K;
                    for (int k = 0; k < K; ++k) g[k] += y[k] - m2;
                    g[K] += s2;
                }
                float* go = gs + ((size_t)i * (rows / inner) + tb) * (K + 1);
                for (int k = 0; k <= K; ++k) go[k] = g[k];
            }
        } else {
            const float vv = v[((size_t)i * rows + r) * vld], mean = sum / (float)K;
            for (int k = 0; k < K; ++k) q[qo + k] = (vv + x[k]) - mean;
        }
    }
}

void launch_dueling_q(const float* a, const float* v, float* q, const float* dq, float* da, float* dv, int n, int T, int B, int inner, int K,
                      hipStream_t stream, int ld, int merged, float* gs) {
    const size_t total = (size_t)n * T * B * inner;
    if (ld <= 0) ld = K;
    if (dq) hipLaunchKernelGGL(k_dueling_q<true>, dim3(grid_for(total)), dim3(256), 0, stream, a, v, q, dq, da, dv, n, T, B, inner, K, ld, merged, gs);
    else hipLaunchKernelGGL(k_dueling_q<false>, dim3(grid_for(total)), dim3(256), 0, stream, a, v, q, dq, da, dv, n, T, B, inner, K, ld, merged, gs);
}

struct GatherTable { ssd_row_gather f[SSD_COPY_BLOCKS_MAX]; };
typedef uint32_t u32_unaligned __attribute__((aligned(1)));
__global__ __launch_bounds__(256) void k_gather_rows(GatherTable t, const int64_t* __restrict__ ids) {
    const ssd_row_gather f = t.f[blockIdx.y];
    const uint8_t* src = static_cast<const uint8_t*>(f.src) + (size_t)ids[blockIdx.z] * f.row_bytes;
    uint8_t* dst = static_cast<uint8_t*>(f.dst) + (size_t)blockIdx.z * f.row_bytes;
    const long words = f.row_bytes >> 2;
    for (long i = (long)blockIdx.x * 256 + threadIdx.x; i < words; i += (long)gridDim.x * 256)
        *reinterpret_cast<u32_unaligned*>(dst + 4 * i) = *reinterpret_cast<const u32_unaligned*>(src + 4 * i);
    if (blockIdx.x == 0 && (long)threadIdx.x < (f.row_bytes & 3)) dst[4 * words + threadIdx.x] = src[4 * words + threadIdx.x];
}

void launch_gather_rows(const ssd_row_gather* fields, int count, const int64_t* ids, int n_ids, hipStream_t stream) {
    GatherTable t;
    int64_t most = 4;
    for (int i = 0; i < SSD_COPY_BLOCKS_MAX; ++i) {
        t.f[i] = fields[i < count ? i : 0];
        if (i < count && fields[i].row_bytes > most) most = fields[i].row_bytes;
    }
    int gx = (int)((most / 4 + 1023) / 1024);
    if (gx < 1) gx = 1;
    if (gx > 32) gx = 32;
    hipLaunchKernelGGL(k_gather_rows, dim3(gx, count, n_ids), dim3(256), 0, stream, t, ids);
}

__device__ __forceinline__ uint32_t sample_draw(uint32_t s0, uint32_t s1, uint32_t call, uint32_t i) {
    uint32_t x = s0 ^ (call * 0x9E3779B9u);
    x ^= x >> 17; x *= 0xed5ad4bbu; x ^= x >> 11; x *= 0xac4c1b51u; x ^= x >> 15; x *= 0x31848babu; x ^= x >> 14;
    x ^= s1 + i * 0x85EBCA6Bu;
    x ^= x >> 17; x *= 0xed5ad4bbu; x ^= x >> 11; x *= 0xac4c1b51u; x ^= x >> 15; x *= 0x31848babu; x ^= x >> 14;
    return x;
}
template <int S>
__global__ __launch_bounds__(64) void k_sample_draw(uint32_t s0, uint32_t s1, uint32_t call, int population, int count, int n_starts,
                                                    int64_t* __restrict__ ids, int64_t* __restrict__ t0) {
    __shared__ int32_t tv[SSD_SAMPLE_IDS_MAX], kv[SSD_SAMPLE_IDS_MAX];
    if (blockIdx.x != 0) return;
    const int lane = threadIdx.x;
    for (int i = lane; i < count; i += 64) {
        tv[i] = (int)(((uint64_t)sample_draw(s0, s1, call, (uint32_t)i) * (uint32_t)(population - count + i + 1)) >> 32);
        kv[i] = (int)(((uint64_t)sample_draw(s0, s1, call, (uint32_t)(count + i)) * (uint32_t)(i + 1)) >> 32);
        if (t0) t0[i] = (int64_t)(((uint64_t)sample_draw(s0, s1, call, (uint32_t)(2 * count + i)) * (uint32_t)n_starts) >> 32);
    }
    __syncthreads();
    int32_t p[S];
#pragma unroll
    for (int s = 0; s < S; ++s) p[s] = -1;
    int t = tv[0];
    for (int i = 0; i < count; ++i) {
        const int t_next = tv[i + 1 < count ? i + 1 : i];
        bool found = false;
#pragma unroll
        for (int s = 0; s < S; ++s) found |= p[s] == t;
        const int v = __ballot(found) ? population - count + i : t;
#pragma unroll
        for (int s = 0; s < S; ++s)
            if (s == (i >> 6) && lane == (i & 63)) p[s] = v;
        t = t_next;
    }
    int k = kv[count - 1];
    for (int i = count - 1; i > 0; --i) {
        const int k_next = kv[i - 1];
        const int ku = __builtin_amdgcn_readfirstlane(k);
        int va = 0, vb = 0;
#pragma unroll
        for (int s = 0; s < S; ++s) {
            va = s == (i >> 6) ? p[s] : va;
            vb = s == (ku >> 6) ? p[s] : vb;
        }
        const int a = __builtin_amdgcn_readlane(va, i & 63), b = __builtin_amdgcn_readlane(vb, ku & 63);
#pragma unroll
        for (int s = 0; s < S; ++s) {
            if (s == (i >> 6) && lane == (i & 63)) p[s] = b;
            if (s == (ku >> 6) && lane == (ku & 63)) p[s] = a;
        }
        k = k_next;
    }
#pragma unroll
    for (int s = 0; s < S; ++s)
        if (s * 64 + lane < count) ids[s * 64 + lane] = (int64_t)p[s];
}
// ... 817 lines not shown
```

homophily_marl_amd/learners/homophily_learner.py:

```python
import os
from collections.abc import Mapping
from types import SimpleNamespace

import numpy as np
import torch as th
import torch.distributed as dist
from torch.optim import Adam

from .. import ops
from ..components.episode_buffer import EpisodeBatch
from ..controllers import REGISTRY as mac_REGISTRY

NEG = -9999999


def validate_target_tau(raw):
    try:
        tau = 0.0 if raw is None else float(raw)
    except (TypeError, ValueError):
        tau = float("nan")
    if isinstance(raw, bool) or not 0.0 <= tau <= 1.0:
        raise ValueError("target_tau must be a finite number in [0, 1], got %r" % (raw,))
    return tau

# ... 37 lines not shown
    def __iter__(self):
        return iter(self.KEYS)

    def __len__(self):
        return len(self.KEYS)

    def host_items(self, extra=(), gap=None):
        with th.no_grad():
            flat = th.cat([self.sums.detach().float().reshape(-1), self.dens.detach().float().reshape(-1)] + [v.detach().float().reshape(1) for _, v in extra]
                          + ([] if gap is None else [gap.detach().float().reshape(-1)]))
        host = flat.cpu()
        ns = self.sums.numel()
        host_logs = _FusedLogs(host[:ns], host[ns:ns + self.dens.numel()], self.rows, self.n)
        out = [(k, float(host[ns + self.dens.numel() + i])) for i, (k, _) in enumerate(extra)]
        if gap is not None:
            out.append(("target_gap_rel", gap_rel(host[ns + self.dens.numel() + len(extra):])))
        return out + [(k, float(host_logs[k])) for k in self.KEYS]

    def synced(self):
        s = self.sums.detach().clone()
        dist.all_reduce(s, op=dist.ReduceOp.SUM)
        return _FusedLogs(s, self.dens, self.rows * dist.get_world_size(), self.n)


class HomophilyLearner:
    def __init__(self, mac, scheme, logger, args):
        self.args, self.mac, self.logger = args, mac, logger
        self.device = args.device
        self.n_agents = n = args.n_agents
        self.n_actions = args.n_actions
        eye = th.eye(n)
        self.inc_mask = (1 - eye).reshape(1, 1, n, n).to(self.device)
        self.env_sim_mask = (1 - eye).reshape(1, 1, n, n, 1).to(self.device)
        self.inc_sim_mask = (1 - eye).reshape(1, 1, n, 1, n).to(self.device)
        self.oth_sim_mask = (1 - eye).reshape(1, 1, 1, n, n).to(self.device)
        self.sim_horizon = args.sim_horizon
        lam = float(getattr(args, "td_lambda", 0.0) or 0.0)
        if not 0.0 <= lam <= 1.0:
            raise ValueError("td_lambda must lie in [0, 1], got %r" % (getattr(args, "td_lambda", None),))
        self.per = (float(getattr(args, "per_alpha", 0.6)), float(getattr(args, "per_eta", 0.9)), float(getattr(args, "per_eps", 1e-3)))
        self.params = list(mac.parameters())
        self.params_env = mac.parameters_env()
        self.params_inc = mac.parameters_inc()
        self.last_target_update_episode = 0
        self.target_tau = validate_target_tau(getattr(args, "target_tau", 0.0))
        self._polyak = None
        self._gap_partials = None
        self._gap_lazy = False
        if self.target_tau > 0 and logger is not None and getattr(logger, "console_logger", None) is not None:
            logger.console_logger.info("target_tau %g: the target network follows the live one after every train step; "
                                       "target_update_interval (%s) is ignored" % (self.target_tau, getattr(args, "target_update_interval", None)))
        on_gpu = str(self.device).startswith("cuda")
        self.use_graph = bool(getattr(args, "train_graph", False)) and on_gpu
        self.fused_adam = on_gpu and bool(getattr(args, "fused_adam", True))
        self.optimiser_env = Adam(params=self.params_env, lr=args.lr_env, capturable=self.use_graph, fused=self.fused_adam or None)
        self.optimiser_inc = Adam(params=self.params_inc, lr=args.lr_inc, capturable=self.use_graph, fused=self.fused_adam or None)
        self._flat_grad = None
        self._graph = None
        self._opt_plan = None
        self._static_batch = None
        self._graph_calls = 0
        self.target_mac = mac_REGISTRY[args.mac](scheme, None, args)
        self.target_mac.load_state(mac)
        for p in self.target_mac.parameters():
            p.requires_grad_(False)
        self.log_stats_t = -self.args.learner_log_interval - 1
        self.log_clock = None
        self.distributed = dist.is_available() and dist.is_initialized() and (dist.get_world_size() > 1 or
                                                                               os.environ.get("SSD_FORCE_DIST") == "1")
        self.profile_collectives = False
        self._coll_events, self._coll_wall = [], []
        ld = str(getattr(args, "learner_dtype", "fp32")).lower()
        if ld not in ("fp32", "float32", "bf16", "bfloat16"):
            raise ValueError("learner_dtype must be fp32 or bf16, got %r" % (ld,))
        self.precision = 1 if ld in ("bf16", "bfloat16") else 2

    @staticmethod
    def unroll(mac, batch):
        return mac.unroll(batch)

    def unroll_pair(self, batch):
        mac, tgt = self.mac, self.target_mac
        shared = mac.unroll_shared(batch)
        gi, wh, bh = mac.unroll_pre(batch, shared)
        with th.no_grad():
            gi_t, wh_t, bh_t = tgt.unroll_pre(batch, shared)
        h0 = mac.stored_h0(batch)
        he, hi, he_t, hi_t = ops.gru_sequence_parts(list(gi) + list(gi_t), batch.max_seq_length, batch.batch_size, list(wh) + list(wh_t), list(bh) + list(bh_t),
                                                    h0=None if h0 is None else h0 + h0)
        if h0 is not None:
            self.last_first_states = (he.detach()[:, 0], hi.detach()[:, 0])
        q_env, q_inc = mac.agent.unroll_post(he, hi, shared["other"])
        with th.no_grad():
            tq_env, tq_inc = tgt.agent.unroll_post(he_t.detach(), hi_t.detach(), shared["other"])
        return q_env, q_inc, tq_env, tq_inc

    def _all_reduce_grad(self):
        if not self.profile_collectives:
            dist.all_reduce(self._flat_grad, op=dist.ReduceOp.SUM)
            return
        import time
        t0 = time.perf_counter()
        ev = None
        if self._flat_grad.is_cuda:
            ev = (th.cuda.Event(enable_timing=True), th.cuda.Event(enable_timing=True))
            ev[0].record()
        dist.all_reduce(self._flat_grad, op=dist.ReduceOp.SUM)
        if ev is not None:
            ev[1].record()
            self._coll_events.append(ev)
        self._coll_wall.append(time.perf_counter() - t0)

    def collective_times(self, reset=True):
        out = dict(calls=len(self._coll_wall))
        if self._coll_events:
            th.cuda.synchronize()
            ms = [a.elapsed_time(b) for a, b in self._coll_events]
            out.update(device_ms_avg=sum(ms) / len(ms), device_ms_max=max(ms))
        if self._coll_wall:
            out["host_ms_avg"] = 1e3 * sum(self._coll_wall) / len(self._coll_wall)
        if reset:
            self._coll_events, self._coll_wall = [], []
        return out

    def _global(self, x):
        if self.distributed:
            x = x.clone()
            dist.all_reduce(x, op=dist.ReduceOp.SUM)
        return x

    def _sim_inputs(self, batch):
        a, n, h = self.args, self.n_agents, self.sim_horizon
        rewards = batch["reward"][:, :-1] / a.reward_scale
        clean_num = (batch["clean_num"][:, :-1] > 0).float()
        cn_cum, rw_cum = th.cumsum(clean_num, dim=1), th.cumsum(rewards, dim=1)
        cn_h, rw_h = cn_cum.clone(), rw_cum.clone()
        cn_h[:, h:] -= cn_cum[:, :-h]
        rw_h[:, h:] -= rw_cum[:, :-h]
        clean_num_t, rewards_t = (cn_h > 0).float(), (rw_h > 0).float()
        which_cluster = 2 * rewards_t + clean_num_t
        is_idle = clean_num_t + rewards_t
        idle_agent = (is_idle.unsqueeze(2) * is_idle.unsqueeze(3)).unsqueeze(-1)
        similarity = (which_cluster.unsqueeze(2) == which_cluster.unsqueeze(3)).unsqueeze(-1).float() * idle_agent
        return th.relu(similarity) * self.env_sim_mask * self.inc_sim_mask * self.oth_sim_mask

    def _td_mask(self, batch):
        terminated = batch["terminated"][:, :-1].float()
        mask = batch["filled"][:, :-1].float()
        mask[:, 1:] = mask[:, 1:] * (1 - terminated[:, :-1])
        return mask.expand(-1, -1, self.n_agents)

    def _fused(self, batch):
        return bool(getattr(self.args, "fused_loss", True)) and batch["reward"].is_cuda and self.n_agents >= 2

    def denominators(self, batch):
        if self._fused(batch):
            d = ops.loss_denominators(batch, self.args, self.n_actions)
        else:
            d = th.stack([self._td_mask(batch).sum(), self._sim_inputs(batch).sum()])
        if self.distributed:
            dist.all_reduce(d, op=dist.ReduceOp.SUM)
        return d

    def _bind_flat_grad(self):
        if self._flat_grad is None:
            self._flat_grad = th.zeros(sum(p.numel() for p in self.params), dtype=th.float32, device=self.params[0].device)
            off = 0
            for p in self.params:
                p.grad = self._flat_grad[off:off + p.numel()].view_as(p)
                off += p.numel()

    def _backward(self, loss, seeds=None):
        self._bind_flat_grad()
        if getattr(self.args, "grad_by_cat", True):
            grads = th.autograd.grad(loss, self.params, grad_outputs=seeds)
            th.cat([g.reshape(-1) for g in grads], out=self._flat_grad)
        else:
# ... 381 lines not shown
```

homophily_marl_amd/modules/agents/homophily_agent.py:

```python
import math

import torch as th
import torch.nn as nn
import torch.nn.functional as F

from ... import ops


class HomophilyAgent(nn.Module):
    def __init__(self, input_shape, args):
        super().__init__()
        self.args = args
        self.n_agents = n = args.n_agents
        self.n_actions = args.n_actions
        self.n_inc_actions = args.n_inc_actions
        self.input_shape = input_shape
        self.hidden = H = args.rnn_hidden_dim
        self.extra_input_shape = args.n_actions + 2 + 2 + 3
        self._gru_cache = None
        self._fc2_cache = None
        if args.rgb_input:
            k = args.conv_kernel
            flat = args.conv_out * (args.obs_dims[0] - k + 1) * (args.obs_dims[1] - k + 1)
            self.conv_to_fc = nn.Sequential(nn.Conv2d(3, args.conv_out, k, args.conv_stride), nn.LeakyReLU(), nn.Flatten(),
# ... 71 lines not shown
    def _gru_weights(self, head):
        return self._gru_weights_both()[0 if head == "env" else 1]

    def _gru_weights_both(self):
        frozen = not self.rnn_env_ir_w.requires_grad
        if frozen:
            if self._gru_cache is None:
                got = {h: self._gru_weights_cat(h) for h in ("env", "inc")}
                if th.is_grad_enabled():
                    return got["env"], got["inc"]
                self._gru_cache = got
            return self._gru_cache["env"], self._gru_cache["inc"]
        groups = []
        for head in ("env", "inc"):
            p = "rnn_%s_" % head
            groups += [[self._w(p + g + "_w") for g in ("ir", "iz", "in")], [self._w(p + g + "_w") for g in ("hr", "hz", "hn")],
                       [self._b(p + g + "_b") for g in ("ir", "iz", "in")], [self._b(p + g + "_b") for g in ("hr", "hz", "hn")]]
        out = ops.cat_groups(groups)
        return tuple(out[:4]), tuple(out[4:])

    def _gru_weights_cat(self, head):
        p = "rnn_%s_" % head
        wi = th.cat([self._w(p + "ir_w"), self._w(p + "iz_w"), self._w(p + "in_w")], dim=2)
        wh = th.cat([self._w(p + "hr_w"), self._w(p + "hz_w"), self._w(p + "hn_w")], dim=2)
        bi = th.cat([self._b(p + "ir_b"), self._b(p + "iz_b"), self._b(p + "in_b")], dim=2)
        bh = th.cat([self._b(p + "hr_b"), self._b(p + "hz_b"), self._b(p + "hn_b")], dim=2)
        return wi, wh, bi, bh

    def load_state_dict(self, *args, **kwargs):
        out = super().load_state_dict(*args, **kwargs)
        if self._gru_cache is not None:
            with th.no_grad():
                for h, bufs in self._gru_cache.items():
                    for dst, src in zip(bufs, self._gru_weights_cat(h)):
                        dst.copy_(src)
        if self._fc2_cache is not None:
            with th.no_grad():
                bufs, self._fc2_cache = self._fc2_cache, None
                for dst, src in zip(bufs, self._fc2_merged()):
                    dst.copy_(src)
                self._fc2_cache = bufs
        return out

    def _apply(self, fn, *args, **kwargs):
        self._gru_cache = None
        self._fc2_cache = None
        return super()._apply(fn, *args, **kwargs)

    def cache_slices(self):
        out = []

        def slices(buf, names):
            col = 0
            for name in names:
                out.append((name, buf, col))
                col += getattr(self, name).shape[-1]
            assert col == buf.shape[-1] and buf.is_contiguous(), names
        if self._gru_cache is not None:
            for head, (wi, wh, bi, bh) in self._gru_cache.items():
                p = "rnn_%s_" % head
                for buf, gates, kind in ((wi, ("ir", "iz", "in"), "_w"), (wh, ("hr", "hz", "hn"), "_w"), (bi, ("ir", "iz", "in"), "_b"), (bh, ("hr", "hz", "hn"), "_b")):
                    slices(buf, [p + g + kind for g in gates])
        if self._fc2_cache is not None:
            for buf, names in zip(self._fc2_cache, (("fc2_env_w", "fc2_env_v_w"), ("fc2_env_b", "fc2_env_v_b"), ("fc2_inc_w", "fc2_inc_v_w"), ("fc2_inc_b", "fc2_inc_v_b"))):
                slices(buf, names)
        return out

    def unroll(self, inputs, act_onehot, agent_pos, agent_orientation, reward, clean_num, apple_den):
        parts, wh, bh = self.unroll_pre(inputs, act_onehot)
        he, hi = ops.gru_sequence_parts(parts, inputs.shape[1], inputs.shape[0], wh, bh)
        return self.unroll_post(he, hi, self.unroll_other(act_onehot, agent_pos, agent_orientation, reward, clean_num, apple_den, inputs.dtype))

    def unroll_pre(self, inputs, act_onehot, act_tm=None):
        B, T, n = inputs.shape[0], inputs.shape[1], self.n_agents
        H = self.hidden
        tm = lambda x: x.permute(2, 1, 0, 3).reshape(n, T * B, x.shape[-1])
        x = tm(inputs)
        act = act_tm if act_tm is not None else tm(act_onehot.to(inputs.dtype))
        xe = ops.bias_bmm(x, self._w("fc1_env_w"), self._b("fc1_env_b"), leaky=True)
        xi = ops.bias_bmm(th.cat([x, act], dim=-1), self._w("fc1_inc_w"), self._b("fc1_inc_b"), leaky=True)
        (wie, whe, bie, bhe), (wii, whi, bii, bhi) = self._gru_weights_both()
        return [ops.bias_bmm(xe, wie, bie), ops.bias_bmm(xi, wii, bii)], [whe, whi], [bhe, bhi]

    @staticmethod
    def unroll_other(act_onehot, agent_pos, agent_orientation, reward, clean_num, apple_den, dtype):
        T, B, n = act_onehot.shape[1], act_onehot.shape[0], act_onehot.shape[2]
        return th.cat([act_onehot.to(dtype), agent_pos, agent_orientation, reward.unsqueeze(-1), clean_num.unsqueeze(-1),
                       apple_den.unsqueeze(-1)], dim=-1).permute(1, 0, 2, 3).reshape(T * B, n, -1)

    def _fc2_merged(self):
        frozen = not self.fc2_env_w.requires_grad
        if frozen and self._fc2_cache is not None:
            return self._fc2_cache
        groups = [[self._w("fc2_env_w"), self._w("fc2_env_v_w")], [self._b("fc2_env_b"), self._b("fc2_env_v_b")],
                  [self._w("fc2_inc_w"), self._w("fc2_inc_v_w")], [self._b("fc2_inc_b"), self._b("fc2_inc_v_b")]]
        out = tuple(ops.cat_groups(groups))
        if frozen and not th.is_grad_enabled():
            self._fc2_cache = out
        return out

    def unroll_post(self, he, hi, other):
        n, H = self.n_agents, self.hidden
        T, B = he.shape[1], he.shape[2]
        he, hi = he.reshape(n, T * B, H), hi.reshape(n, T * B, H)
        w_env, b_env, w_inc, b_inc = self._fc2_merged()
        q_env = ops.dueling_head(he, None, w_env, b_env, B, T, 1)
        q_inc = ops.dueling_head(hi, other, w_inc, b_inc, B, T, n)
        return q_env, q_inc

    def forward_env(self, inputs, h_in, learning_mode=False):
        n, H = self.n_agents, self.hidden
        x = inputs.reshape(-1, n, self.input_shape).transpose(0, 1)
        h = h_in.reshape(-1, n, H).transpose(0, 1)
        x = F.leaky_relu(th.baddbmm(self._b("fc1_env_b"), x, self._w("fc1_env_w")))
        h_out = self._gru("env", x, h)
        a = th.baddbmm(self._b("fc2_env_b"), h_out, self._w("fc2_env_w"))
        v = th.baddbmm(self._b("fc2_env_v_b"), h_out, self._w("fc2_env_v_w"))
        q = v + a - a.mean(dim=-1, keepdim=True)
        return q.transpose(0, 1), h_out.transpose(0, 1).unsqueeze(2), {}

    def forward_inc(self, inputs, h_in, actions_env, agent_pos, agent_orientation, reward, clean_num, apple_den,
                    learning_mode=False):
        n, H = self.n_agents, self.hidden
        act = actions_env.reshape(-1, n, self.n_actions).to(inputs.dtype)
        B = act.shape[0]
        x = th.cat([inputs.reshape(B, n, self.input_shape), act], dim=-1).transpose(0, 1)
        h = h_in.reshape(B, n, H).transpose(0, 1)
        x = F.leaky_relu(th.baddbmm(self._b("fc1_inc_b"), x, self._w("fc1_inc_w")))
        h_out = self._gru("inc", x, h)
        other = th.cat([act, agent_pos.reshape(B, n, 2), agent_orientation.reshape(B, n, 2), reward.reshape(B, n, 1),
                        clean_num.reshape(B, n, 1), apple_den.reshape(B, n, 1)], dim=-1)
        E = other.shape[-1]
        cat = th.cat([h_out.unsqueeze(2).expand(n, B, n, H), other.unsqueeze(0).expand(n, B, n, E)], dim=-1)
        cat = cat.reshape(n, B * n, H + E)
        a = th.baddbmm(self._b("fc2_inc_b"), cat, self._w("fc2_inc_w"))
        v = th.baddbmm(self._b("fc2_inc_v_b"), cat, self._w("fc2_inc_v_w"))
        q = (v + a - a.mean(dim=-1, keepdim=True)).reshape(n, B, n, -1).transpose(0, 1)
        return q, h_out.transpose(0, 1).unsqueeze(2), {}
```

homophily_marl_amd/ops.py:

```python
import ctypes as C

import torch as th

from . import abi


def _stream(t):
    return th.cuda.current_stream(t.device).cuda_stream


import os as _os
STRICT = _os.environ.get("SSD_STRICT_DEVICE_OPS") == "1"


def numeric_status():
    lib = abi.load_library()
    bits = C.c_int32(0)
    abi.check(lib, lib.ssd_numeric_status(C.byref(bits)))
    return bits.value


def reserve_bmm_scratch(stream):
    lib = abi.load_library()
    abi.check(lib, lib.ssd_bmm_reserve_scratch(stream.cuda_stream))
# ... 340 lines not shown
        da = th.empty(n, T * B * inner, K, dtype=th.float32, device=dq.device)
        dv = th.empty(n, T * B * inner, 1, dtype=th.float32, device=dq.device)
        abi.check(lib, lib.ssd_dueling_q_bwd(dq.data_ptr(), da.data_ptr(), dv.data_ptr(), n, T, B, inner, K, _stream(dq)))
        return da, dv, None, None, None


def dueling_q(a, v, B, T, inner):
    n, K = a.shape[0], a.shape[-1]
    if a.dim() != 3 or a.shape[1] != T * B * inner:
        raise _unfit("dueling_q", "a", a, "[n, T * B * inner = %d, K] expected" % (T * B * inner))
    if v.shape != (n, T * B * inner, 1) or v.device != a.device:
        raise _unfit("dueling_q", "v", v, "%s on the device of a expected" % ((n, T * B * inner, 1),))
    if a.is_cuda and _f32_on(a, v) and K <= 16:
        q = _DuelingQ.apply(a, v, B, T, inner)
    else:
        _leaving_kernels("dueling_q", a, "K = %d > 16 or dtypes %s, %s" % (K, a.dtype, v.dtype))
        q = (v + a - a.mean(dim=-1, keepdim=True)).reshape(n, T, B, inner, K).permute(2, 1, 0, 3, 4)
    return q.reshape(B, T, n, K) if inner == 1 else q


class _DuelingHead(th.autograd.Function):

    @staticmethod
    def forward(ctx, h, other, w, b, B, T, inner):
        lib = abi.load_library()
        h, w, b = h.contiguous(), w.contiguous(), b.contiguous()
        n, TB, H = h.shape
        K = w.shape[2] - 1
        st = _stream(h)
        y = th.empty(n, TB * inner, K + 1, dtype=th.float32, device=h.device)
        if other is None:
            assert inner == 1 and w.shape[1] == H
            abi.check(lib, lib.ssd_bias_bmm_fwd(h.data_ptr(), w.data_ptr(), b.data_ptr(), y.data_ptr(), n, TB, H, K + 1, st))
        else:
            other = other.contiguous()
            E = other.shape[-1]
            assert other.shape[0] == TB and other.shape[1] == inner and w.shape[1] == H + E
            abi.check(lib, lib.ssd_bias_bmm2_fwd(h.data_ptr(), other.data_ptr(), w.data_ptr(), b.data_ptr(), y.data_ptr(), n, TB * inner, H, E, K + 1,
                                                 inner, 1, st))
        q = th.empty((B, T, n, inner, K), dtype=th.float32, device=h.device)
        abi.check(lib, lib.ssd_dueling_head_fwd(y.data_ptr(), q.data_ptr(), n, T, B, inner, K, st))
        ctx.save_for_backward(h, w, *(() if other is None else (other,)))
        ctx.dims = (B, T, inner, K)
        ctx.precision = LEARNER_PRECISION
        return q

    @staticmethod
    def backward(ctx, dq):
        with _precision(ctx.precision):
            return _DuelingHead._backward(ctx, dq)

    @staticmethod
    def _backward(ctx, dq):
        lib = abi.load_library()
        h, w = ctx.saved_tensors[:2]
        other = ctx.saved_tensors[2] if len(ctx.saved_tensors) > 2 else None
        B, T, inner, K = ctx.dims
        n, TB, H = h.shape
        st = _stream(h)
        dq = dq.contiguous()
        need = ctx.needs_input_grad
        dy = th.empty(n, TB * inner, K + 1, dtype=th.float32, device=h.device)
        two = other is not None
        gs = th.empty(n, TB, K + 1, dtype=th.float32, device=h.device) if (two and need[0]) else None
        abi.check(lib, lib.ssd_dueling_head_bwd(dq.data_ptr(), dy.data_ptr(), None if gs is None else gs.data_ptr(), n, T, B, inner, K, st))
        dw = th.empty_like(w) if need[2] else None
        db = th.empty(n, 1, K + 1, dtype=th.float32, device=h.device) if need[3] else None
        ptr = lambda t: None if t is None else t.data_ptr()
        dh = None
        if not two:
            dh = th.empty_like(h) if need[0] else None
            abi.check(lib, lib.ssd_bias_bmm_bwd(dy.data_ptr(), h.data_ptr(), w.data_ptr(), ptr(dh), ptr(dw), ptr(db), None, n, TB, H, K + 1, st))
        else:
            E = other.shape[-1]
            if dw is not None or db is not None:
                abi.check(lib, lib.ssd_bias_bmm2_bwd_w(dy.data_ptr(), h.data_ptr(), other.data_ptr(), ptr(dw), ptr(db), n, TB * inner, H, E, K + 1, inner, 1, st))
            if need[0]:
                dh = th.empty_like(h)
                abi.check(lib, lib.ssd_bias_bmm_bwd_x(gs.data_ptr(), w.data_ptr(), dh.data_ptr(), n, TB, H, K + 1, (H + E) * (K + 1), st))
        assert not need[1]
        return dh, None, dw, db, None, None, None


def dueling_head(h, other, w, b, B, T, inner):
    if h.dim() != 3 or h.shape[1] != T * B:
        raise _unfit("dueling_head", "h", h, "[n, T * B = %d, H] expected" % (T * B))
    n, TB, H = h.shape
    if other is not None and (other.dim() != 3 or tuple(other.shape[:2]) != (TB, inner) or other.device != h.device):
        raise _unfit("dueling_head", "other", other, "[T * B = %d, inner = %d, E] on the device of h expected" % (TB, inner))
    E = 0 if other is None else other.shape[-1]
    if w.dim() != 3 or tuple(w.shape[:2]) != (n, H + E) or w.shape[2] < 2 or w.device != h.device:
        raise _unfit("dueling_head", "w", w, "[n = %d, H (+ E) = %d, K + 1] on the device of h expected" % (n, H + E))
    K = w.shape[2] - 1
    if b.device != h.device:
        raise _unfit("dueling_head", "b", b, "the device of h expected")
    if (h.is_cuda and _f32_on(h, w, b) and K <= 15 and H % 16 == 0 and b.shape == (n, 1, K + 1) and (other is not None or inner == 1)
            and (other is None or (other.dtype == th.float32 and E >= 1 and not (other.requires_grad and th.is_grad_enabled())))):
        q = _DuelingHead.apply(h, other, w, b, B, T, inner)
    else:
        _leaving_kernels("dueling_head", h, "layout / dtypes / a bias that is not [n, 1, K + 1] / other requires a gradient")
        x = h if other is None else th.cat([h.unsqueeze(2).expand(n, TB, inner, h.shape[-1]), other.unsqueeze(0).expand(n, TB, inner, other.shape[-1])],
                                          dim=-1).reshape(n, TB * inner, -1)
        y = _baddbmm(b, x, w)
        a, v = y[..., :K], y[..., K:]
        q = (v + a - a.mean(dim=-1, keepdim=True)).reshape(n, T, B, inner, K).permute(2, 1, 0, 3, 4)
    return q.reshape(B, T, n, K) if inner == 1 else q


def _mix32p(x):
    x &= 0xFFFFFFFF
    x ^= x >> 17; x = (x * 0xed5ad4bb) & 0xFFFFFFFF; x ^= x >> 11; x = (x * 0xac4c1b51) & 0xFFFFFFFF
    x ^= x >> 15; x = (x * 0x31848bab) & 0xFFFFFFFF; x ^= x >> 14
    return x


def _sample_draw(seed, call, i):
    s0, s1 = seed & 0xFFFFFFFF, (seed >> 32) & 0xFFFFFFFF
    x = _mix32p(s0 ^ ((call * 0x9E3779B9) & 0xFFFFFFFF))
    return _mix32p(x ^ ((s1 + i * 0x85EBCA6B) & 0xFFFFFFFF))


def sample_ids(seed, call, population, count, out):
    assert out.dtype == th.long and out.numel() >= count and 1 <= count <= population
    if out.is_cuda:
        lib = abi.load_library()
        abi.check(lib, lib.ssd_sample_ids(seed & (2 ** 64 - 1), call & 0xFFFFFFFF, population, count, out.data_ptr(), _stream(out)))
        return out
    ids = []
    for i in range(count):
        j = population - count + i
        t = (_sample_draw(seed, call & 0xFFFFFFFF, i) * (j + 1)) >> 32
        ids.append(j if t in ids else t)
    for i in range(count - 1, 0, -1):
        k = (_sample_draw(seed, call & 0xFFFFFFFF, count + i) * (i + 1)) >> 32
        ids[i], ids[k] = ids[k], ids[i]
    out[:count] = th.tensor(ids, dtype=th.long)
    return out


def gather_rows(pairs, ids):
    if not pairs or len(pairs) > abi.COPY_BLOCKS_MAX or not ids.is_cuda or ids.dtype != th.long:
        return False
    n = ids.numel()
    if n < 1 or n > 65535:
        return False
    for src, dst in pairs:
        if not (src.is_cuda and dst.is_cuda and src.is_contiguous() and dst.is_contiguous() and src.dtype == dst.dtype
                and dst.shape[0] == n and dst.shape[1:] == src.shape[1:] and src[0].numel() > 0):
            return False
    lib = abi.load_library()
    tab = (abi.SsdRowGather * len(pairs))()
    for e, (src, dst) in zip(tab, pairs):
        e.src, e.dst, e.row_bytes = src.data_ptr(), dst.data_ptr(), src[0].numel() * src.element_size()
    abi.check(lib, lib.ssd_gather_rows(tab, len(pairs), ids.contiguous().data_ptr(), n, _stream(ids)))
    return True


def sample_windows(seed, call, population, count, n_starts, ids_out, t0_out):
    assert ids_out.dtype == th.long and t0_out.dtype == th.long and ids_out.numel() >= count and t0_out.numel() >= count
    assert 1 <= count <= population and n_starts >= 1 and ids_out.is_cuda == t0_out.is_cuda
    if ids_out.is_cuda:
        assert ids_out.is_contiguous() and t0_out.is_contiguous()
        lib = abi.load_library()
        abi.check(lib, lib.ssd_sample_windows(seed & (2 ** 64 - 1), call & 0xFFFFFFFF, population, count, n_starts, ids_out.data_ptr(),
                                              t0_out.data_ptr(), _stream(ids_out)))
        return ids_out, t0_out
    sample_ids(seed, call, population, count, ids_out)
    t0_out[:count] = th.tensor([(_sample_draw(seed, call & 0xFFFFFFFF, 2 * count + e) * n_starts) >> 32 for e in range(count)], dtype=th.long)
    return ids_out, t0_out


def gather_windows(pairs, ids, t0, src_slots, win_slots, burn_in, filled_index):
    if not pairs or len(pairs) > abi.COPY_BLOCKS_MAX or not (ids.is_cuda and t0.is_cuda) or ids.dtype != th.long or t0.dtype != th.long:
        return False
    n = ids.numel()
    if n < 1 or n > 65535 or t0.numel() != n or not 2 <= win_slots <= src_slots or not 0 <= burn_in <= win_slots - 2:
        return False
    for k, (src, dst) in enumerate(pairs):
        if not (src.is_cuda and dst.is_cuda and src.is_contiguous() and dst.is_contiguous() and src.dtype == dst.dtype and src.dim() >= 2
                and src.shape[1] == src_slots and tuple(dst.shape[:2]) == (n, win_slots) and dst.shape[2:] == src.shape[2:] and src[0, 0].numel() > 0):
            return False
        if k == filled_index and not (src.dtype == th.long and src[0, 0].numel() == 1):
            return False
    lib = abi.load_library()
    tab = (abi.SsdWindowField * len(pairs))()
    for k, (e, (src, dst)) in enumerate(zip(tab, pairs)):
        e.src, e.dst, e.slot_bytes, e.filled = src.data_ptr(), dst.data_ptr(), src[0, 0].numel() * src.element_size(), int(k == filled_index)
    abi.check(lib, lib.ssd_gather_windows(tab, len(pairs), ids.contiguous().data_ptr(), t0.contiguous().data_ptr(), n, src_slots, win_slots,
                                          burn_in, _stream(ids)))
# ... 231 lines not shown
        grads = full
        flat = th.empty(sum(int(th.Size(sh).numel()) for sh in ctx.shapes), dtype=th.float32, device=dev)
        res, entries, k, off = [], [], 0, 0
        for cnt, g in zip(ctx.sizes, grads):
            total, col = g.shape[-1], 0
            for sh in ctx.shapes[k:k + cnt]:
                c, numel = sh[-1], int(th.Size(sh).numel())
                d = flat[off:off + numel]
                entries.append((g.data_ptr() + 4 * col, d.data_ptr(), numel // c, c, total, c))
                res.append(d.view(sh))
                col += c
                off += numel
            k += cnt
        _copy_blocks(entries, flat)
        return (None,) + tuple(res)


def cat_groups(groups):
    flat = [t for g in groups for t in g]
    if (flat[0].is_cuda and len(flat) <= abi.COPY_BLOCKS_MAX and all(t.dtype == th.float32 and t.is_cuda for t in flat)
            and all(t.shape[:-1] == g[0].shape[:-1] for g in groups for t in g)):
        return list(_CatGroups.apply(tuple(len(g) for g in groups), *flat))
    _leaving_kernels("cat_groups", flat[0], "%d tensors / dtypes / leading axes" % len(flat))
    return [th.cat(list(g), dim=-1) for g in groups]


def _baddbmm(b, x, w):
    dt = th.promote_types(th.promote_types(b.dtype, x.dtype), w.dtype)
    return th.baddbmm(b.to(dt), x.to(dt), w.to(dt))


def _bmm_kernel_ok(x, w, b):
    return (x.is_cuda and x.dim() == 3 and w.dim() == 3 and _f32_on(x, w, b) and w.shape[0] == x.shape[0] and w.shape[1] == x.shape[2]
            and b.shape == (x.shape[0], 1, w.shape[2]))


def _bias_bmm_fwd(x, w, b, leaky=False):
    lib = abi.load_library()
    x, w, b = x.contiguous(), w.contiguous(), b.contiguous()
    n, R, I = x.shape
    O = w.shape[2]
    y = th.empty(n, R, O, dtype=th.float32, device=x.device)
    fn = lib.ssd_bias_bmm_leaky_fwd if leaky else lib.ssd_bias_bmm_fwd
    abi.check(lib, fn(x.data_ptr(), w.data_ptr(), b.data_ptr(), y.data_ptr(), n, R, I, O, _stream(x)))
    return y


class _BiasBmm(th.autograd.Function):

    @staticmethod
    def forward(ctx, x, w, b, leaky):
        x, w = x.contiguous(), w.contiguous()
        y = _bias_bmm_fwd(x, w, b, leaky)
        ctx.leaky = leaky
        ctx.precision = LEARNER_PRECISION
        ctx.save_for_backward(x, w, *((y,) if leaky else ()))
        return y

    @staticmethod
    def backward(ctx, g):
        with _precision(ctx.precision):
            return _BiasBmm._backward(ctx, g)

    @staticmethod
    def _backward(ctx, g):
        lib = abi.load_library()
        x, w = ctx.saved_tensors[:2]
        g = g.contiguous()
        n, R, I = x.shape
        O = w.shape[2]
        need = ctx.needs_input_grad
        dx = th.empty_like(x) if need[0] else None
        dw = th.empty_like(w) if need[1] else None
        db = th.empty(n, 1, O, dtype=th.float32, device=x.device) if need[2] else None
        ptr = lambda t: None if t is None else t.data_ptr()
        if ctx.leaky:
            y = ctx.saved_tensors[2]
            abi.check(lib, lib.ssd_bias_bmm_leaky_bwd(g.data_ptr(), y.data_ptr(), x.data_ptr(), w.data_ptr(), ptr(dx), ptr(dw), ptr(db), None, n, R, I, O, _stream(x)))
        else:
            abi.check(lib, lib.ssd_bias_bmm_bwd(g.data_ptr(), x.data_ptr(), w.data_ptr(), ptr(dx), ptr(dw), ptr(db), None, n, R, I, O, _stream(x)))
        return dx, dw, db, None


def bias_bmm(x, w, b, leaky=False):
    if _bmm_kernel_ok(x, w, b):
        if th.is_grad_enabled() and (w.requires_grad or b.requires_grad or x.requires_grad):
            return _BiasBmm.apply(x, w, b, leaky)
        return _bias_bmm_fwd(x, w, b, leaky)
    if x.dim() != 3:
        raise _unfit("bias_bmm", "x", x, "[n, R, I] expected")
    if w.dim() != 3 or tuple(w.shape[:2]) != (x.shape[0], x.shape[2]) or w.device != x.device:
        raise _unfit("bias_bmm", "w", w, "[n = %d, I = %d, O] on the device of x expected" % (x.shape[0], x.shape[2]))
    if b.device != x.device:
        raise _unfit("bias_bmm", "b", b, "the device of x expected")
    _leaving_kernels("bias_bmm", x, "dtypes %s, %s, %s / a bias that is not [n, 1, O]" % (x.dtype, w.dtype, b.dtype))
    y = _baddbmm(b, x, w)
    return th.nn.functional.leaky_relu(y) if leaky else y


class _BiasLinear(th.autograd.Function):

    @staticmethod
    def forward(ctx, x, w, b):
        ctx.save_for_backward(x, w)
        return th.addmm(b, x, w.t())

    @staticmethod
    def backward(ctx, g):
        x, w = ctx.saved_tensors
        g = g.contiguous()
        return (g @ w if ctx.needs_input_grad[0] else None, g.t() @ x if ctx.needs_input_grad[1] else None,
                column_sums(g) if ctx.needs_input_grad[2] else None)


class _ChannelBias(th.autograd.Function):

    @staticmethod
    def forward(ctx, y, b):
        return y + b.view(1, -1, 1, 1)

    @staticmethod
    def backward(ctx, g):
        R, C = g.shape[0], g.shape[1]
        db = column_sums(column_sums(g.reshape(R, -1)).view(C, -1).t().contiguous()) if ctx.needs_input_grad[1] else None
        return g, db


def channel_bias(y, b):
    return _ChannelBias.apply(y, b)


def bias_linear(x, w, b):
    if x.is_cuda and (w.requires_grad or b.requires_grad or x.requires_grad):
        return _BiasLinear.apply(x, w, b)
    return th.nn.functional.linear(x, w, b)


def expand_codes(codes):
    c = codes.unsqueeze(-3)
    return th.cat([c == 2, c == 1, c == 3], dim=-3).float() * (255.0 / 256.0)


def encode_codes_supported(codes):
    return codes.is_cuda and codes.dtype == th.uint8 and codes.shape[-1] == codes.shape[-2] and abi.encode_edge_supported(codes.shape[-1])


class _EncodeCodes(th.autograd.Function):

    @staticmethod
    def forward(ctx, codes, conv_w, conv_b, lin_w, lin_b):
        lib = abi.load_library()
        codes = codes.contiguous()
        R, V = codes.shape[0], codes.shape[-1]
        O = V - 2
        dev = codes.device
        st = _stream(codes)
        cw, lw = conv_w.detach().contiguous(), lin_w.detach().contiguous()
        cb, lb = conv_b.detach().contiguous(), lin_b.detach().contiguous()
        prec = LEARNER_PRECISION
        need = any(ctx.needs_input_grad[1:])
        layout = abi.ENCODE_LAYOUT_TOEPLITZ if need and V in (15, 31) else abi.ENCODE_LAYOUT_LUT
        cbytes, lbytes = abi.encode_frag_bytes(V, prec, layout)
        cf, lf = th.empty(cbytes, dtype=th.uint8, device=dev), th.empty(lbytes, dtype=th.uint8, device=dev)
        pack = lib.ssd_policy_pack_encoder if layout == abi.ENCODE_LAYOUT_TOEPLITZ else lib.ssd_policy_pack_encoder_lut
        abi.check(lib, pack(cw.data_ptr(), cb.data_ptr(), lw.data_ptr(), V, prec, cf.data_ptr(), lf.data_ptr(), st))
        act = th.empty(R, 6, O, O, dtype=th.float32, device=dev) if need else None
        bands = abi.encode_bands(V)
        ea = abi.SsdPolicyEncodeArgs()
        ea.codes, ea.code_bytes = codes.data_ptr(), codes.numel()
        ea.env_stride, ea.slot_stride, ea.agent_stride, ea.slot_t = V * V, 0, V * V, None
        ea.rows, ea.view_edge, ea.n_agents, ea.agent_major, ea.precision = R, V, 1, 0, prec
        ea.layout = layout
        ea.alphabet = abi.CODE_CLASS
        ea.conv_frags, ea.lin_frags, ea.conv_b, ea.lin_b = cf.data_ptr(), lf.data_ptr(), cb.data_ptr(), lb.data_ptr()
        ea.act = None if act is None else act.data_ptr()
        if bands == 1:
            feat = th.empty(R, 32, dtype=th.float32, device=dev)
            ea.out, ea.out_stride = feat.data_ptr(), 32
            abi.check(lib, lib.ssd_policy_encode(C.byref(ea), st))
        else:
            part = th.empty(bands, R, 32, dtype=th.float32, device=dev)
            ea.part = part.data_ptr()
            abi.check(lib, lib.ssd_policy_encode(C.byref(ea), st))
            feat = th.nn.functional.leaky_relu(column_sums(part.view(bands, R * 32)).view(R, 32) + lb)
        if need:
            ctx.save_for_backward(codes, act, feat, cw, lw)
        ctx.precision = prec
        return feat

    @staticmethod
    def backward(ctx, d_feat):
        with _precision(ctx.precision):
            return _EncodeCodes._backward(ctx, d_feat)

    @staticmethod
    def _backward(ctx, d_feat):
        lib = abi.load_library()
        codes, act, feat, cw, lw = ctx.saved_tensors
        R = codes.shape[0]
        K = act[0].numel()
        st = _stream(codes)
        g2 = th.ops.aten.leaky_relu_backward(d_feat.contiguous(), feat, 0.01, True)
        d_lin_b = column_sums(g2)
        d_lin_w = th.empty(32, K, dtype=th.float32, device=codes.device)
        abi.check(lib, lib.ssd_bias_bmm_bwd(act.data_ptr(), g2.data_ptr(), None, None, d_lin_w.data_ptr(), None, None, 1, R, 32, K, st))
        d_act = th.empty_like(act)
        lwt = lw.t().contiguous()
        abi.check(lib, lib.ssd_bias_bmm_bwd(g2.data_ptr(), None, lwt.data_ptr(), d_act.data_ptr(), None, None, act.data_ptr(), 1, R, K, 32, st))
        P = lib.ssd_conv_wgrad_partial_rows(R)
        part = th.empty(P, 168, dtype=th.float32, device=codes.device)
        abi.check(lib, lib.ssd_conv_wgrad_codes(codes.data_ptr(), d_act.data_ptr(), part.data_ptr(), R, codes.shape[-1], st))
        tot = column_sums(part)
        return None, tot[:162].view(cw.shape), tot[162:], d_lin_w, d_lin_b


def encode_codes(codes, conv_w, conv_b, lin_w, lin_b):
    if codes.dim() != 3 or codes.shape[-1] != codes.shape[-2] or codes.shape[-1] < 3:
        raise _unfit("encode_codes", "codes", codes, "[R, V, V] with V >= 3 expected")
    K = 6 * (codes.shape[-1] - 2) ** 2
    for name, t, shape in (("conv_w", conv_w, (6, 3, 3, 3)), ("conv_b", conv_b, (6,)), ("lin_w", lin_w, (32, K)), ("lin_b", lin_b, (32,))):
        if t.shape != shape or t.device != codes.device:
            raise _unfit("encode_codes", name, t, "%s on the device of codes expected" % (shape,))
    if encode_codes_supported(codes) and _f32_on(conv_w, conv_b, lin_w, lin_b):
        return _EncodeCodes.apply(codes, conv_w, conv_b, lin_w, lin_b)
    _leaving_kernels("encode_codes", codes, "dtype %s / edge %d" % (codes.dtype, codes.shape[-1]))
    act = th.nn.functional.leaky_relu(th.nn.functional.conv2d(expand_codes(codes).to(conv_w.dtype), conv_w, conv_b))
    return th.nn.functional.leaky_relu(th.nn.functional.linear(act.flatten(1), lin_w, lin_b))


class _GruGates(th.autograd.Function):

    @staticmethod
    def forward(ctx, gi, gh, h):
        lib = abi.load_library()
        gi, gh, h = gi.contiguous(), gh.contiguous(), h.contiguous()
        R, H = h.numel() // h.shape[-1], h.shape[-1]
        h_new, rzn = th.empty_like(h), th.empty_like(gi)
        abi.check(lib, lib.ssd_gru_gates_fwd(gi.data_ptr(), gh.data_ptr(), h.data_ptr(), h_new.data_ptr(), rzn.data_ptr(), R, H, _stream(h)))
        ctx.save_for_backward(rzn, gh, h)
        return h_new

    @staticmethod
    def backward(ctx, dh):
        lib = abi.load_library()
        rzn, gh, h = ctx.saved_tensors
        dh = dh.contiguous()
        R, H = h.numel() // h.shape[-1], h.shape[-1]
        d_gi, d_gh, dh_prev = th.empty_like(rzn), th.empty_like(rzn), th.empty_like(h)
        abi.check(lib, lib.ssd_gru_gates_bwd(dh.data_ptr(), rzn.data_ptr(), gh.data_ptr(), h.data_ptr(), d_gi.data_ptr(), d_gh.data_ptr(),
                                             dh_prev.data_ptr(), R, H, _stream(h)))
        return d_gi, d_gh, dh_prev


class _GruSeq(th.autograd.Function):

    @staticmethod
    def forward(ctx, gi, wh, bh, h0):
        lib = abi.load_library()
        gi, wh, bh = gi.contiguous(), wh.contiguous(), bh.contiguous()
        T, G, B, H3 = gi.shape
        H = H3 // 3
        Bp = (B + 15) // 16 * 16
        if Bp != B:
            gi = th.nn.functional.pad(gi, (0, 0, 0, Bp - B))
        hs = th.empty(G, T, Bp, H, dtype=gi.dtype, device=gi.device)
        need = any(ctx.needs_input_grad)
        rzn = th.empty_like(gi) if need else None
        ghn = th.empty(T, G, Bp, H, dtype=gi.dtype, device=gi.device) if need else None
        if h0 is None:
            abi.check(lib, lib.ssd_gru_seq_fwd(gi.data_ptr(), wh.data_ptr(), bh.data_ptr(), hs.data_ptr(), None if rzn is None else rzn.data_ptr(),
                                               None if ghn is None else ghn.data_ptr(), T, G, Bp, _stream(gi)))
        else:
            h0 = h0.contiguous() if Bp == B else th.nn.functional.pad(h0, (0, 0, 0, Bp - B))
            one = lambda t: (C.c_void_p * 1)(t.data_ptr())
            abi.check(lib, lib.ssd_gru_seq_fwd_h0(one(gi), 0, one(wh), one(bh), 1, one(h0), Bp * H, H, hs.data_ptr(), None if rzn is None else rzn.data_ptr(),
                                                  None if ghn is None else ghn.data_ptr(), T, G, Bp, _stream(gi)))
        ctx.h0 = h0 is not None
        if need:
            ctx.save_for_backward(hs, rzn, ghn, wh)
            ctx.B = B
        ctx.precision = LEARNER_PRECISION
        return hs if Bp == B else hs[:, :, :B].contiguous()

    @staticmethod
    def backward(ctx, dhs):
# ... 216 lines not shown
```

Before: 347.8 million.

## Batch online and target network forward passes into paired kernel launches

Adds paired kernels that run the learner's online and frozen target networks' bias-bmm and dueling-head forwards in a single grid, split by blockIdx.y. A new fc1_rows kernel builds the time-major fc1 inputs for both nets, with and without actions, in one pass, along with a matching backward kernel. The aim is to cut kernel launch count and the separate cat/permute copies in the training step. The cost is more ABI surface and extra code paths that only engage when shapes and frozen-target conditions match.

```diff
diff --git a/__graft_entry__.py b/__graft_entry__.py
--- a/__graft_entry__.py
+++ b/__graft_entry__.py
@@ -7,7 +7,7 @@
     sys.path.insert(0, ROOT)
 
 CSRC = os.path.join(ROOT, "homophily_marl_amd", "csrc")
-HIP_SOURCES = ["ssd_env.hip", "ssd_learner.hip", "ssd_policy.hip", "ssd_policy_mfma.hip", "ssd_gru_seq.hip", "ssd_bmm.hip", "ssd_abi.hip"]
+HIP_SOURCES = ["ssd_env.hip", "ssd_learner.hip", "ssd_policy.hip", "ssd_policy_mfma.hip", "ssd_gru_seq.hip", "ssd_bmm.hip", "ssd_train_rows.hip", "ssd_abi.hip"]
 HIP_LIB = os.path.join(ROOT, "homophily_marl_amd", "libssd_hip.so")
 HIPCC_FLAGS = ["--offload-arch=gfx950", "-O3", "-std=c++17", "-fPIC", "-shared", "-ffp-contract=off",
                "-fno-fast-math", "-Wall", "-Wno-unused-function", "-mllvm", "-amdgpu-kernarg-preload-count=14"]
@@ -22,7 +22,7 @@
 
 def build(force=False):
     srcs = [os.path.join(CSRC, s) for s in HIP_SOURCES]
-    hdrs = [os.path.join(CSRC, h) for h in os.listdir(CSRC) if h.endswith(".h")] + [os.path.join(ROOT, "include", "ssd_hip.h")]
+    hdrs = [os.path.join(CSRC, h) for h in os.listdir(CSRC) if h.endswith(".h")] + [os.path.join(ROOT, "include", h) for h in ("ssd_hip.h", "ssd_hip_train.h")]
     if force or _stale(HIP_LIB, srcs + hdrs + [os.path.abspath(__file__)]):
         from concurrent.futures import ThreadPoolExecutor
         hipcc = os.environ.get("HIPCC", "/opt/rocm/bin/hipcc")
diff --git a/homophily_marl_amd/abi.py b/homophily_marl_amd/abi.py
--- a/homophily_marl_amd/abi.py
+++ b/homophily_marl_amd/abi.py
@@ -323,6 +323,12 @@
     "ssd_numeric_status": [P(i32)],
 }.items()}
 HIP_SIGNATURES.update(_sigs("ssd_", True))
+TRAIN_SIGNATURES = {name: (C.c_int, args) for name, args in {
+    "ssd_bias_bmm_pair_fwd": [vp] * 5 + [i32] + [vp] * 5 + [i32] * 8 + [vp],
+    "ssd_dueling_head_pair_fwd": [vp, vp, i32, vp, vp, i32] + [i32] * 4 + [vp],
+    "ssd_fc1_rows_fwd": [vp] * 8 + [i32] * 6 + [vp],
+    "ssd_fc1_rows_bwd": [vp] * 3 + [i32] * 7 + [vp],
+}.items()}
 
 
 def onehot_rows(n_agents, n_actions, flags):
@@ -461,6 +467,7 @@
                 "(hipcc --offload-arch=gfx950).  There is no CPU fallback." % HIP_LIB_PATH)
         lib = C.CDLL(HIP_LIB_PATH)
         bind(lib, HIP_SIGNATURES)
+        bind(lib, TRAIN_SIGNATURES)
         ver = lib.ssd_abi_version()
         if ver != ABI_VERSION:
             raise ImportError("libssd_hip.so ABI version %d != %d" % (ver, ABI_VERSION))
diff --git a/homophily_marl_amd/controllers/homophily_controller.py b/homophily_marl_amd/controllers/homophily_controller.py
--- a/homophily_marl_amd/controllers/homophily_controller.py
+++ b/homophily_marl_amd/controllers/homophily_controller.py
@@ -196,20 +196,39 @@
         return sh
 
     def unroll_pre(self, batch, shared):
+        return self.agent.unroll_pre(self.unroll_inputs(batch, shared), shared["onehot"], act_tm=shared.get("act_tm"))
+
+    def unroll_feat(self, batch, shared):
         a = self.args
         B, T, n = batch.batch_size, batch.max_seq_length, self.n_agents
         obs = shared["obs"]
         if shared.get("codes") is not None:
-            feat = self.agent.rgb_preprocess_codes(shared["codes"].reshape(B * T * n, a.obs_dims[0], a.obs_dims[1]))
-        elif a.rgb_input:
-            feat = self.agent.rgb_preprocess(obs.reshape(B * T * n, 3, a.obs_dims[0], a.obs_dims[1]))
-        else:
-            feat = obs.reshape(B * T * n, -1)
+            return self.agent.rgb_preprocess_codes(shared["codes"].reshape(B * T * n, a.obs_dims[0], a.obs_dims[1]))
+        if a.rgb_input:
+            return self.agent.rgb_preprocess(obs.reshape(B * T * n, 3, a.obs_dims[0], a.obs_dims[1]))
+        return obs.reshape(B * T * n, -1)
+
+    def unroll_inputs(self, batch, shared):
+        B, T, n = batch.batch_size, batch.max_seq_length, self.n_agents
+        feat = self.unroll_feat(batch, shared)
         if shared["tail"] is not None:
-            inputs = th.cat([feat, shared["tail"]], dim=1).reshape(B, T, n, -1)
-        else:
-            inputs = self.assemble_inputs(feat, *shared["hist"], False).reshape(B, T, n, -1)
-        return self.agent.unroll_pre(inputs, shared["onehot"], act_tm=shared.get("act_tm"))
+            return th.cat([feat, shared["tail"]], dim=1).reshape(B, T, n, -1)
+        return self.assemble_inputs(feat, *shared["hist"], False).reshape(B, T, n, -1)
+
+    def unroll_rows_pair(self, tgt, batch, shared):
+        B, T, n = batch.batch_size, batch.max_seq_length, self.n_agents
+        if shared["tail"] is not None and shared.get("act_tm") is not None:
+            feat = self.unroll_feat(batch, shared)
+            with th.no_grad():
+                feat_t = tgt.unroll_feat(batch, shared)
+            return ops.fc1_rows(feat, shared["tail"], shared["act_tm"], B, T, n, feat_t)
+        tm = lambda x: x.permute(2, 1, 0, 3).reshape(n, T * B, x.shape[-1])
+        x = tm(self.unroll_inputs(batch, shared))
+        act = shared["act_tm"] if shared.get("act_tm") is not None else tm(shared["onehot"].to(x.dtype))
+        with th.no_grad():
+            x_t = tm(tgt.unroll_inputs(batch, shared))
+            xa_t = th.cat([x_t, act], dim=-1)
+        return x, th.cat([x, act], dim=-1), x_t, xa_t
 
     def _build_inputs(self, batch, t):
         if self.args.rgb_input:
diff --git a/homophily_marl_amd/csrc/ssd_abi.hip b/homophily_marl_amd/csrc/ssd_abi.hip
--- a/homophily_marl_amd/csrc/ssd_abi.hip
+++ b/homophily_marl_amd/csrc/ssd_abi.hip
@@ -5,6 +5,7 @@
 #include <vector>
 
 #include "ssd_device.h"
+#include "../../include/ssd_hip_train.h"
 
 using namespace ssd;
 
@@ -851,6 +852,50 @@
     if (!g || !w || !dx || n < 1 || rows < 1 || in < 1 || out < 1 || w_set < (int64_t)in * out) return fail(SSD_ERR_INVALID, "bad argument");
     if (launch_bias_bmm_bwd(g, nullptr, w, dx, nullptr, nullptr, nullptr, n, rows, in, out, (hipStream_t)stream, 0, 0, nullptr, nullptr, 0, 1, 0, (long)w_set))
         return fail(SSD_ERR_UNSUPPORTED, "ssd_bias_bmm_bwd_x: an operand set of 2^30 elements or more");
+    return launched();
+}
+int ssd_bias_bmm_pair_fwd(const float* x_a, const float* x2_a, const float* w_a, const float* b_a, float* y_a, int32_t n_a, const float* x_b,
+                          const float* x2_b, const float* w_b, const float* b_b, float* y_b, int32_t n_b, int32_t rows, int32_t in1, int32_t in2,
+                          int32_t out, int32_t x1_div, int32_t x2_shared, int32_t leaky, void* stream) {
+    if (!x_a || !w_a || !b_a || !y_a || !x_b || !w_b || !b_b || !y_b) return fail(SSD_ERR_INVALID, "ssd_bias_bmm_pair_fwd: a null operand of either group");
+    if (n_a < 1 || n_b < 1) return fail(SSD_ERR_INVALID, "ssd_bias_bmm_pair_fwd: both groups need a set count >= 1");
+    if (rows < 1 || in1 < 1 || in2 < 0 || out < 1) return fail(SSD_ERR_INVALID, "ssd_bias_bmm_pair_fwd: bad argument");
+    if ((in2 > 0) != (x2_a != nullptr) || (in2 > 0) != (x2_b != nullptr))
+        return fail(SSD_ERR_INVALID, "ssd_bias_bmm_pair_fwd: in2 > 0 needs the second source of both groups, in2 == 0 neither");
+    if ((long)n_a + n_b > 65535) return fail(SSD_ERR_UNSUPPORTED, "ssd_bias_bmm_pair_fwd: more than 65535 weight sets in one grid");
+    const int rc = launch_bias_bmm_pair_fwd(x_a, x2_a, w_a, b_a, y_a, n_a, x_b, x2_b, w_b, b_b, y_b, n_b, rows, in1, in2, out, x1_div, x2_shared, leaky != 0,
+                                            (hipStream_t)stream);
+    if (rc == -3)
+        return fail(SSD_ERR_INVALID, "ssd_bias_bmm_pair_fwd: rows a multiple of x1_div >= 1; in1 a multiple of 16 unless in2 is no multiple of 4");
+    if (rc) return fail(SSD_ERR_UNSUPPORTED, "ssd_bias_bmm_pair_fwd: a weight / operand set of 2^30 elements or more");
+    return launched();
+}
+int ssd_dueling_head_pair_fwd(const float* y_a, float* q_a, int32_t n_a, const float* y_b, float* q_b, int32_t n_b, int32_t T, int32_t B, int32_t inner,
+                              int32_t K, void* stream) {
+    if (!y_a || !q_a || !y_b || !q_b) return fail(SSD_ERR_INVALID, "ssd_dueling_head_pair_fwd: a null operand of either group");
+    if (n_a < 1 || n_b < 1) return fail(SSD_ERR_INVALID, "ssd_dueling_head_pair_fwd: both groups need a set count >= 1");
+    if (T < 1 || B < 1 || inner < 1 || K < 1 || K > 15) return fail(SSD_ERR_INVALID, "ssd_dueling_head_pair_fwd: bad argument");
+    launch_dueling_q(y_a, y_a + K, q_a, nullptr, nullptr, nullptr, n_a, T, B, inner, K, (hipStream_t)stream, K + 1, 1, nullptr, y_b, y_b + K, q_b, n_b);
+    return launched();
+}
+int ssd_fc1_rows_fwd(const float* feat_a, const float* feat_b, const float* tail, const float* act, float* x_env_a, float* x_inc_a, float* x_env_b,
+                     float* x_inc_b, int32_t B, int32_t T, int32_t n, int32_t feat_w, int32_t tail_w, int32_t act_w, void* stream) {
+    if (!feat_a || !act || !x_env_a || !x_inc_a) return fail(SSD_ERR_INVALID, "ssd_fc1_rows_fwd: a null operand of the first net");
+    if ((feat_b != nullptr) != (x_env_b != nullptr) || (feat_b != nullptr) != (x_inc_b != nullptr))
+        return fail(SSD_ERR_INVALID, "ssd_fc1_rows_fwd: the second net's features and both its outputs come together or not at all");
+    if (B < 1 || T < 1 || n < 1 || feat_w < 1 || tail_w < 0 || act_w < 1) return fail(SSD_ERR_INVALID, "ssd_fc1_rows_fwd: bad argument");
+    if ((tail_w > 0) != (tail != nullptr)) return fail(SSD_ERR_INVALID, "ssd_fc1_rows_fwd: tail_w > 0 needs tail, tail_w == 0 none");
+    if ((int64_t)B * T * n * ((int64_t)feat_w + tail_w + act_w) >= ((int64_t)1 << 40)) return fail(SSD_ERR_UNSUPPORTED, "ssd_fc1_rows_fwd: 2^40 elements or more");
+    launch_fc1_rows(feat_a, feat_b, tail, act, x_env_a, x_inc_a, x_env_b, x_inc_b, B, T, n, feat_w, tail_w, act_w, (hipStream_t)stream);
+    return launched();
+}
+int ssd_fc1_rows_bwd(const float* d_x_env, const float* d_x_inc, float* d_feat, int32_t B, int32_t T, int32_t n, int32_t feat_w, int32_t tail_w, int32_t act_w,
+                     int32_t d_feat_stride, void* stream) {
+    if (!d_x_env || !d_x_inc || !d_feat) return fail(SSD_ERR_INVALID, "ssd_fc1_rows_bwd: a null operand");
+    if (B < 1 || T < 1 || n < 1 || feat_w < 1 || tail_w < 0 || act_w < 1) return fail(SSD_ERR_INVALID, "ssd_fc1_rows_bwd: bad argument");
+    if (d_feat_stride < feat_w) return fail(SSD_ERR_INVALID, "ssd_fc1_rows_bwd: d_feat_stride below feat_w");
+    if ((int64_t)B * T * n * ((int64_t)feat_w + tail_w + act_w) >= ((int64_t)1 << 40)) return fail(SSD_ERR_UNSUPPORTED, "ssd_fc1_rows_bwd: 2^40 elements or more");
+    launch_fc1_rows_bwd(d_x_env, d_x_inc, d_feat, B, T, n, feat_w, tail_w, act_w, d_feat_stride, (hipStream_t)stream);
     return launched();
 }
 int ssd_bmm_reserve_scratch(void* stream) {
diff --git a/homophily_marl_amd/csrc/ssd_bmm.hip b/homophily_marl_amd/csrc/ssd_bmm.hip
--- a/homophily_marl_amd/csrc/ssd_bmm.hip
+++ b/homophily_marl_amd/csrc/ssd_bmm.hip
@@ -21,6 +21,7 @@
     long w_set;
     float* part;
     int row_chunks;
+    const float *x_b, *x2_b, *w_b, *b_b; float* y_b; int n_a;
 };
 constexpr int BMM_PART = 272;
 
@@ -57,20 +58,24 @@
     const int otiles = (O + 15) >> 4, groups = (otiles + BMM_TPW - 1) / BMM_TPW, rtiles = (R + 15) >> 4;
     const int unit = blockIdx.x * 4 + wave;
     if (unit >= rtiles * groups) return;
-    const int g = blockIdx.y, row0 = (unit / groups) * 16, t0 = (unit % groups) * BMM_TPW;
+    const int row0 = (unit / groups) * 16, t0 = (unit % groups) * BMM_TPW;
     const int rowc = row0 + m < R ? row0 + m : R - 1;
+    const bool grp_b = a.n_a && (int)blockIdx.y >= a.n_a;
+    const int g = grp_b ? blockIdx.y - a.n_a : blockIdx.y;
+    const float *ax = grp_b ? a.x_b : a.x, *ax2 = grp_b ? a.x2_b : a.x2, *aw = grp_b ? a.w_b : a.w, *ab = grp_b ? a.b_b : a.b;
+    float* ay = grp_b ? a.y_b : a.y;
     const bool two = a.x2 != nullptr;
     const int I1 = two ? a.I1 : I;
-    const float* xs = a.x + (two ? (size_t)g * (size_t)(R / a.x1_div) * I1 : (size_t)g * R * I);
+    const float* xs = ax + (two ? (size_t)g * (size_t)(R / a.x1_div) * I1 : (size_t)g * R * I);
     const uint32_t xrow = two ? (uint32_t)(rowc / a.x1_div) * (uint32_t)I1 : (uint32_t)rowc * (uint32_t)I;
-    const float* x2s = two ? a.x2 + (size_t)g * a.x2_set : a.x;
+    const float* x2s = two ? ax2 + (size_t)g * a.x2_set : ax;
     const uint32_t x2row = (uint32_t)rowc * (uint32_t)(I - I1);
-    const float* wg = a.w + (size_t)g * (a.w_set ? a.w_set : (long)I * O);
+    const float* wg = aw + (size_t)g * (a.w_set ? a.w_set : (long)I * O);
     f32x4 acc[BMM_TPW];
 #pragma unroll
     for (int t = 0; t < BMM_TPW; ++t) {
         const int o = 16 * (t0 + t) + m;
-        const float bv = (t0 + t < otiles && o < O) ? a.b[(size_t)g * O + o] : 0.f;
+        const float bv = (t0 + t < otiles && o < O) ? ab[(size_t)g * O + o] : 0.f;
         acc[t] = f32x4{bv, bv, bv, bv};
     }
     const int chunks = (I + 15) >> 4;
@@ -152,7 +157,7 @@
         for (int r = 0; r < 4; ++r) {
             const int row = row0 + 4 * q + r;
             const float v = acc[t][r];
-            if (row < R) a.y[((size_t)g * R + row) * O + o] = (a.leaky && !(v > 0.f)) ? 0.01f * v : v;
+            if (row < R) ay[((size_t)g * R + row) * O + o] = (a.leaky && !(v > 0.f)) ? 0.01f * v : v;
         }
     }
 }
@@ -410,6 +415,32 @@
     return 0;
 }
 
+int launch_bias_bmm_pair_fwd(const float* x_a, const float* x2_a, const float* w_a, const float* b_a, float* y_a, int n_a, const float* x_b,
+                             const float* x2_b, const float* w_b, const float* b_b, float* y_b, int n_b, int R, int I1, int I2, int O, int x1_div,
+                             int x2_shared, int leaky, hipStream_t s) {
+    BmmK k = {};
+    const int I = I1 + I2;
+    bool xv = (I & 3) == 0;
+    if (I2) {
+        xv = (I2 & 3) == 0;
+        if (x1_div < 1 || R % x1_div || (xv && (I1 & 15))) return -3;
+        k.x2 = x2_a; k.x2_b = x2_b; k.I1 = I1; k.x1_div = x1_div; k.x2_set = x2_shared ? 0 : (long)R * I2;
+    }
+    if ((long)I * O >= (1L << 30) || (long)R * I >= (1L << 30)) return -2;
+    k.x = x_a; k.w = w_a; k.b = b_a; k.y = y_a; k.x_b = x_b; k.w_b = w_b; k.b_b = b_b; k.y_b = y_b; k.n_a = n_a;
+    k.n = n_a + n_b; k.R = R; k.I = I; k.O = O; k.leaky = leaky;
+    const int otiles = (O + 15) / 16, units = ((R + 15) / 16) * ((otiles + BMM_TPW - 1) / BMM_TPW);
+    const dim3 grid((units + 3) / 4, n_a + n_b);
+    if (g_learner_precision == 1) {
+        if (xv) hipLaunchKernelGGL((k_bias_bmm_fwd<true, true>), grid, dim3(256), 0, s, k);
+        else hipLaunchKernelGGL((k_bias_bmm_fwd<false, true>), grid, dim3(256), 0, s, k);
+    } else {
+        if (xv) hipLaunchKernelGGL((k_bias_bmm_fwd<true, false>), grid, dim3(256), 0, s, k);
+        else hipLaunchKernelGGL((k_bias_bmm_fwd<false, false>), grid, dim3(256), 0, s, k);
+    }
+    return 0;
+}
+
 int launch_bias_bmm_bwd(const float* g, const float* x, const float* w, float* dx, float* dw, float* db, const float* slope_of, int n, int R,
                         int I, int O, hipStream_t s, long x_set, long g_set, const float* act_y, const float* x2, int I1, int x1_div, int x2_shared,
                         long w_set) {
diff --git a/homophily_marl_amd/csrc/ssd_device.h b/homophily_marl_amd/csrc/ssd_device.h
--- a/homophily_marl_amd/csrc/ssd_device.h
+++ b/homophily_marl_amd/csrc/ssd_device.h
@@ -136,7 +136,8 @@
 void launch_copy_blocks(const ssd_block_copy* blocks, int count, hipStream_t stream);
 void launch_clip_adam(const ssd_clip_adam_args* a, hipStream_t stream);
 void launch_dueling_q(const float* a, const float* v, float* q, const float* dq, float* da, float* dv, int n, int T, int B, int inner, int K, hipStream_t stream,
-                      int ld = 0, int merged = 0, float* gs = nullptr);
+                      int ld = 0, int merged = 0, float* gs = nullptr, const float* a_b = nullptr, const float* v_b = nullptr, float* q_b = nullptr,
+                      int n_b = 0);
 void launch_gather_rows(const ssd_row_gather* fields, int count, const int64_t* ids, int n_ids, hipStream_t stream);
 void launch_td_sim_loss(const ssd_td_loss_args* a, int mode, hipStream_t stream);
 constexpr long long kDefaultLdsLimit = 64 * 1024;
@@ -190,6 +191,12 @@
                         int x1_div = 1, int x2_shared = 0, long w_set = 0);
 int launch_bias_bmm2_fwd(const float* x1, const float* x2, const float* w, const float* b, float* y, int n, int R, int I1, int I2, int O, int x1_div,
                          int x2_shared, hipStream_t s);
+int launch_bias_bmm_pair_fwd(const float* x_a, const float* x2_a, const float* w_a, const float* b_a, float* y_a, int n_a, const float* x_b,
+                             const float* x2_b, const float* w_b, const float* b_b, float* y_b, int n_b, int R, int I1, int I2, int O, int x1_div,
+                             int x2_shared, int leaky, hipStream_t s);
+void launch_fc1_rows(const float* feat_a, const float* feat_b, const float* tail, const float* act, float* xe_a, float* xi_a, float* xe_b, float* xi_b, int B,
+                     int T, int n, int F0, int F1, int A, hipStream_t s);
+void launch_fc1_rows_bwd(const float* dxe, const float* dxi, float* d_feat, int B, int T, int n, int F0, int F1, int A, int ld, hipStream_t s);
 #ifdef SSD_STAMPS
 void set_policy_stamps(unsigned long long* buf);
 #endif
diff --git a/homophily_marl_amd/csrc/ssd_learner.hip b/homophily_marl_amd/csrc/ssd_learner.hip
--- a/homophily_marl_amd/csrc/ssd_learner.hip
+++ b/homophily_marl_amd/csrc/ssd_learner.hip
@@ -606,17 +606,21 @@
 template <bool BWD>
 __global__ __launch_bounds__(256) void k_dueling_q(const float* __restrict__ a, const float* __restrict__ v, float* __restrict__ q,
                                                    const float* __restrict__ dq, float* __restrict__ da, float* __restrict__ dv, int n, int T, int B,
-                                                   int inner, int K, int ld, int merged, float* __restrict__ gs) {
+                                                   int inner, int K, int ld, int merged, float* __restrict__ gs, const float* __restrict__ a_b,
+                                                   const float* __restrict__ v_b, float* __restrict__ q_b, int n_a) {
     const long rows = (long)T * B * inner, total = rows * n;
     const int vld = merged ? ld : 1;
     for (long idx = (long)blockIdx.x * 256 + threadIdx.x; idx < total; idx += (long)gridDim.x * 256) {
-        const int i = (int)(idx / rows);
+        int i = (int)(idx / rows);
         const long r = idx - (long)i * rows;
         const long tb = r / inner;
         const int j = (int)(r - tb * inner), t = (int)(tb / B), b = (int)(tb - (long)t * B);
-        const size_t qo = ((((size_t)b * T + t) * n + i) * inner + j) * K, ao = ((size_t)i * rows + r) * ld;
+        const bool grp_b = !BWD && n_a && i >= n_a;
+        const int ng = !BWD && n_a ? (grp_b ? n - n_a : n_a) : n;
+        if (grp_b) i -= n_a;
+        const size_t qo = ((((size_t)b * T + t) * ng + i) * inner + j) * K, ao = ((size_t)i * rows + r) * ld;
         float x[16], sum = 0.f;
-        for (int k = 0; k < K; ++k) { x[k] = BWD ? dq[qo + k] : a[ao + k]; sum += x[k]; }
+        for (int k = 0; k < K; ++k) { x[k] = BWD ? dq[qo + k] : (grp_b ? a_b : a)[ao + k]; sum += x[k]; }
         if (BWD) {
             const float mean = sum / (float)K;
             for (int k = 0; k < K; ++k) da[ao + k] = x[k] - mean;
@@ -636,18 +640,21 @@
                 for (int k = 0; k <= K; ++k) go[k] = g[k];
             }
         } else {
-            const float vv = v[((size_t)i * rows + r) * vld], mean = sum / (float)K;
-            for (int k = 0; k < K; ++k) q[qo + k] = (vv + x[k]) - mean;
+            const float vv = (grp_b ? v_b : v)[((size_t)i * rows + r) * vld], mean = sum / (float)K;
+            float* qg = grp_b ? q_b : q;
+            for (int k = 0; k < K; ++k) qg[qo + k] = (vv + x[k]) - mean;
         }
     }
 }
 
 void launch_dueling_q(const float* a, const float* v, float* q, const float* dq, float* da, float* dv, int n, int T, int B, int inner, int K,
-                      hipStream_t stream, int ld, int merged, float* gs) {
+                      hipStream_t stream, int ld, int merged, float* gs, const float* a_b, const float* v_b, float* q_b, int n_b) {
+    const int n_a = (!dq && n_b > 0) ? n : 0;
+    if (n_a) n += n_b;
     const size_t total = (size_t)n * T * B * inner;
     if (ld <= 0) ld = K;
-    if (dq) hipLaunchKernelGGL(k_dueling_q<true>, dim3(grid_for(total)), dim3(256), 0, stream, a, v, q, dq, da, dv, n, T, B, inner, K, ld, merged, gs);
-    else hipLaunchKernelGGL(k_dueling_q<false>, dim3(grid_for(total)), dim3(256), 0, stream, a, v, q, dq, da, dv, n, T, B, inner, K, ld, merged, gs);
+    if (dq) hipLaunchKernelGGL(k_dueling_q<true>, dim3(grid_for(total)), dim3(256), 0, stream, a, v, q, dq, da, dv, n, T, B, inner, K, ld, merged, gs, a_b, v_b, q_b, n_a);
+    else hipLaunchKernelGGL(k_dueling_q<false>, dim3(grid_for(total)), dim3(256), 0, stream, a, v, q, dq, da, dv, n, T, B, inner, K, ld, merged, gs, a_b, v_b, q_b, n_a);
 }
 
 struct GatherTable { ssd_row_gather f[SSD_COPY_BLOCKS_MAX]; };
diff --git a/homophily_marl_amd/csrc/ssd_train_rows.hip b/homophily_marl_amd/csrc/ssd_train_rows.hip
--- /dev/null
+++ b/homophily_marl_amd/csrc/ssd_train_rows.hip
@@ -0,0 +1,60 @@
+#include <hip/hip_runtime.h>
+#include <stdint.h>
+#include "../../include/ssd_hip.h"
+#include "ssd_device.h"
+
+namespace ssd {
+
+__global__ __launch_bounds__(256) void k_fc1_rows(const float* __restrict__ feat_a, const float* __restrict__ feat_b, const float* __restrict__ tail,
+                                                  const float* __restrict__ act, float* __restrict__ xe_a, float* __restrict__ xi_a,
+                                                  float* __restrict__ xe_b, float* __restrict__ xi_b, int B, int T, int n, int F0, int F1, int A, int nets) {
+    const int W = F0 + F1 + A, We = F0 + F1;
+    const long TB = (long)T * B, per_net = (long)n * TB * W, total = per_net * nets;
+    for (long idx = (long)blockIdx.x * 256 + threadIdx.x; idx < total; idx += (long)gridDim.x * 256) {
+        const int net = (int)(idx / per_net);
+        const long e = idx - net * per_net, row = e / W;
+        const int c = (int)(e - row * W), i = (int)(row / TB);
+        const long tb = row - i * TB;
+        const int t = (int)(tb / B), b = (int)(tb - (long)t * B);
+        const long src = ((long)b * T + t) * n + i;
+        float v;
+        if (c < F0) v = (net ? feat_b : feat_a)[src * F0 + c];
+        else if (c < We) v = tail[src * F1 + (c - F0)];
+        else v = act[row * A + (c - We)];
+        (net ? xi_b : xi_a)[row * W + c] = v;
+        if (c < We) (net ? xe_b : xe_a)[row * We + c] = v;
+    }
+}
+
+__global__ __launch_bounds__(256) void k_fc1_rows_bwd(const float* __restrict__ dxe, const float* __restrict__ dxi, float* __restrict__ d_feat, int B, int T,
+                                                      int n, int F0, int F1, int A, int ld) {
+    const int W = F0 + F1 + A, We = F0 + F1;
+    const long TB = (long)T * B, total = (long)n * TB * F0;
+    for (long idx = (long)blockIdx.x * 256 + threadIdx.x; idx < total; idx += (long)gridDim.x * 256) {
+        const long src = idx / F0;
+        const int c = (int)(idx - src * F0), i = (int)(src % n);
+        const long bt = src / n;
+        const int b = (int)(bt / T), t = (int)(bt - (long)b * T);
+        const long row = (long)i * TB + (long)t * B + b;
+        d_feat[src * ld + c] = dxe[row * We + c] + dxi[row * W + c];
+    }
+}
+
+static int rows_grid(long total) {
+    const long b = (total + 255) / 256;
+    return (int)(b > 16384 ? 16384 : b);
+}
+
+void launch_fc1_rows(const float* feat_a, const float* feat_b, const float* tail, const float* act, float* xe_a, float* xi_a, float* xe_b, float* xi_b, int B,
+                     int T, int n, int F0, int F1, int A, hipStream_t s) {
+    const int nets = feat_b ? 2 : 1;
+    const long total = (long)nets * n * T * B * (F0 + F1 + A);
+    hipLaunchKernelGGL(k_fc1_rows, dim3(rows_grid(total)), dim3(256), 0, s, feat_a, feat_b, tail, act, xe_a, xi_a, xe_b, xi_b, B, T, n, F0, F1, A, nets);
+}
+
+void launch_fc1_rows_bwd(const float* dxe, const float* dxi, float* d_feat, int B, int T, int n, int F0, int F1, int A, int ld, hipStream_t s) {
+    const long total = (long)n * T * B * F0;
+    hipLaunchKernelGGL(k_fc1_rows_bwd, dim3(rows_grid(total)), dim3(256), 0, s, dxe, dxi, d_feat, B, T, n, F0, F1, A, ld);
+}
+
+}
diff --git a/homophily_marl_amd/learners/homophily_learner.py b/homophily_marl_amd/learners/homophily_learner.py
--- a/homophily_marl_amd/learners/homophily_learner.py
+++ b/homophily_marl_amd/learners/homophily_learner.py
@@ -143,17 +143,13 @@
     def unroll_pair(self, batch):
         mac, tgt = self.mac, self.target_mac
         shared = mac.unroll_shared(batch)
-        gi, wh, bh = mac.unroll_pre(batch, shared)
-        with th.no_grad():
-            gi_t, wh_t, bh_t = tgt.unroll_pre(batch, shared)
+        (gi, wh, bh), (gi_t, wh_t, bh_t) = mac.agent.unroll_pre_pair(tgt.agent, *mac.unroll_rows_pair(tgt, batch, shared))
         h0 = mac.stored_h0(batch)
         he, hi, he_t, hi_t = ops.gru_sequence_parts(list(gi) + list(gi_t), batch.max_seq_length, batch.batch_size, list(wh) + list(wh_t), list(bh) + list(bh_t),
                                                     h0=None if h0 is None else h0 + h0)
         if h0 is not None:
             self.last_first_states = (he.detach()[:, 0], hi.detach()[:, 0])
-        q_env, q_inc = mac.agent.unroll_post(he, hi, shared["other"])
-        with th.no_grad():
-            tq_env, tq_inc = tgt.agent.unroll_post(he_t.detach(), hi_t.detach(), shared["other"])
+        (q_env, q_inc), (tq_env, tq_inc) = mac.agent.unroll_post_pair(tgt.agent, he, hi, he_t.detach(), hi_t.detach(), shared["other"])
         return q_env, q_inc, tq_env, tq_inc
 
     def _all_reduce_grad(self):
diff --git a/homophily_marl_amd/modules/agents/homophily_agent.py b/homophily_marl_amd/modules/agents/homophily_agent.py
--- a/homophily_marl_amd/modules/agents/homophily_agent.py
+++ b/homophily_marl_amd/modules/agents/homophily_agent.py
@@ -177,6 +177,27 @@
         (wie, whe, bie, bhe), (wii, whi, bii, bhi) = self._gru_weights_both()
         return [ops.bias_bmm(xe, wie, bie), ops.bias_bmm(xi, wii, bii)], [whe, whi], [bhe, bhi]
 
+    def unroll_pre_pair(self, tgt, x, xa, x_t, xa_t):
+        with th.no_grad():
+            (wie_t, whe_t, bie_t, bhe_t), (wii_t, whi_t, bii_t, bhi_t) = tgt._gru_weights_both()
+        xe, xe_t = ops.bias_bmm_pair(x, self._w("fc1_env_w"), self._b("fc1_env_b"), x_t, tgt._w("fc1_env_w"), tgt._b("fc1_env_b"), leaky=True)
+        xi, xi_t = ops.bias_bmm_pair(xa, self._w("fc1_inc_w"), self._b("fc1_inc_b"), xa_t, tgt._w("fc1_inc_w"), tgt._b("fc1_inc_b"), leaky=True)
+        (wie, whe, bie, bhe), (wii, whi, bii, bhi) = self._gru_weights_both()
+        gie, gie_t = ops.bias_bmm_pair(xe, wie, bie, xe_t, wie_t, bie_t)
+        gii, gii_t = ops.bias_bmm_pair(xi, wii, bii, xi_t, wii_t, bii_t)
+        return ([gie, gii], [whe, whi], [bhe, bhi]), ([gie_t, gii_t], [whe_t, whi_t], [bhe_t, bhi_t])
+
+    def unroll_post_pair(self, tgt, he, hi, he_t, hi_t, other):
+        n, H = self.n_agents, self.hidden
+        T, B = he.shape[1], he.shape[2]
+        he, hi, he_t, hi_t = (h.reshape(n, T * B, H) for h in (he, hi, he_t, hi_t))
+        w_env, b_env, w_inc, b_inc = self._fc2_merged()
+        with th.no_grad():
+            w_env_t, b_env_t, w_inc_t, b_inc_t = tgt._fc2_merged()
+        q_env, tq_env = ops.dueling_head_pair(he, None, w_env, b_env, he_t, w_env_t, b_env_t, B, T, 1)
+        q_inc, tq_inc = ops.dueling_head_pair(hi, other, w_inc, b_inc, hi_t, w_inc_t, b_inc_t, B, T, n)
+        return (q_env, q_inc), (tq_env, tq_inc)
+
     @staticmethod
     def unroll_other(act_onehot, agent_pos, agent_orientation, reward, clean_num, apple_den, dtype):
         T, B, n = act_onehot.shape[1], act_onehot.shape[0], act_onehot.shape[2]
diff --git a/homophily_marl_amd/ops.py b/homophily_marl_amd/ops.py
--- a/homophily_marl_amd/ops.py
+++ b/homophily_marl_amd/ops.py
@@ -446,7 +446,7 @@
         return dh, None, dw, db, None, None, None
 
 
-def dueling_head(h, other, w, b, B, T, inner):
+def _dueling_head_fit(h, other, w, b, B, T, inner):
     if h.dim() != 3 or h.shape[1] != T * B:
         raise _unfit("dueling_head", "h", h, "[n, T * B = %d, H] expected" % (T * B))
     n, TB, H = h.shape
@@ -458,8 +458,14 @@
     K = w.shape[2] - 1
     if b.device != h.device:
         raise _unfit("dueling_head", "b", b, "the device of h expected")
-    if (h.is_cuda and _f32_on(h, w, b) and K <= 15 and H % 16 == 0 and b.shape == (n, 1, K + 1) and (other is not None or inner == 1)
-            and (other is None or (other.dtype == th.float32 and E >= 1 and not (other.requires_grad and th.is_grad_enabled())))):
+    return (h.is_cuda and _f32_on(h, w, b) and K <= 15 and H % 16 == 0 and b.shape == (n, 1, K + 1) and (other is not None or inner == 1)
+            and (other is None or (other.dtype == th.float32 and E >= 1 and not (other.requires_grad and th.is_grad_enabled()))))
+
+
+def dueling_head(h, other, w, b, B, T, inner):
+    fit = _dueling_head_fit(h, other, w, b, B, T, inner)
+    n, TB, K = h.shape[0], h.shape[1], w.shape[2] - 1
+    if fit:
         q = _DuelingHead.apply(h, other, w, b, B, T, inner)
     else:
         _leaving_kernels("dueling_head", h, "layout / dtypes / a bias that is not [n, 1, K + 1] / other requires a gradient")
@@ -469,6 +475,60 @@
         a, v = y[..., :K], y[..., K:]
         q = (v + a - a.mean(dim=-1, keepdim=True)).reshape(n, T, B, inner, K).permute(2, 1, 0, 3, 4)
     return q.reshape(B, T, n, K) if inner == 1 else q
+
+
+class _DuelingHeadPair(th.autograd.Function):
+
+    @staticmethod
+    def forward(ctx, h, other, w, b, B, T, inner, h_t, w_t, b_t):
+        lib = abi.load_library()
+        h, w, b, h_t, w_t, b_t = (t.contiguous() for t in (h, w, b, h_t, w_t, b_t))
+        n, TB, H = h.shape
+        n_t = h_t.shape[0]
+        K = w.shape[2] - 1
+        st = _stream(h)
+        y = th.empty(n, TB * inner, K + 1, dtype=th.float32, device=h.device)
+        y_t = th.empty(n_t, TB * inner, K + 1, dtype=th.float32, device=h.device)
+        if other is None:
+            assert inner == 1 and w.shape[1] == H
+            abi.check(lib, lib.ssd_bias_bmm_pair_fwd(h.data_ptr(), None, w.data_ptr(), b.data_ptr(), y.data_ptr(), n, h_t.data_ptr(), None, w_t.data_ptr(),
+                                                     b_t.data_ptr(), y_t.data_ptr(), n_t, TB, H, 0, K + 1, 1, 0, 0, st))
+        else:
+            other = other.contiguous()
+            E = other.shape[-1]
+            assert other.shape[0] == TB and other.shape[1] == inner and w.shape[1] == H + E
+            abi.check(lib, lib.ssd_bias_bmm_pair_fwd(h.data_ptr(), other.data_ptr(), w.data_ptr(), b.data_ptr(), y.data_ptr(), n, h_t.data_ptr(), other.data_ptr(),
+                                                     w_t.data_ptr(), b_t.data_ptr(), y_t.data_ptr(), n_t, TB * inner, H, E, K + 1, inner, 1, 0, st))
+        q = th.empty((B, T, n, inner, K), dtype=th.float32, device=h.device)
+        q_t = th.empty((B, T, n_t, inner, K), dtype=th.float32, device=h.device)
+        abi.check(lib, lib.ssd_dueling_head_pair_fwd(y.data_ptr(), q.data_ptr(), n, y_t.data_ptr(), q_t.data_ptr(), n_t, T, B, inner, K, st))
+        ctx.save_for_backward(h, w, *(() if other is None else (other,)))
+        ctx.dims = (B, T, inner, K)
+        ctx.precision = LEARNER_PRECISION
+        ctx.mark_non_differentiable(q_t)
+        ctx.set_materialize_grads(False)
+        return q, q_t
+
+    @staticmethod
+    def backward(ctx, dq, dq_t):
+        if dq is None:
+            return (None,) * 10
+        with _precision(ctx.precision):
+            return _DuelingHead._backward(ctx, dq) + (None, None, None)
+
+
+def dueling_head_pair(h, other, w, b, h_t, w_t, b_t, B, T, inner):
+    fit = _dueling_head_fit(h, other, w, b, B, T, inner)
+    frozen = not (th.is_grad_enabled() and (h_t.requires_grad or w_t.requires_grad or b_t.requires_grad))
+    if (fit and frozen and _dueling_head_fit(h_t, other, w_t, b_t, B, T, inner) and h_t.device == h.device
+            and tuple(h_t.shape[1:]) == tuple(h.shape[1:]) and tuple(w_t.shape[1:]) == tuple(w.shape[1:])):
+        q, q_t = _DuelingHeadPair.apply(h, other, w, b, B, T, inner, h_t, w_t, b_t)
+        K = w.shape[2] - 1
+        return (q.reshape(B, T, h.shape[0], K), q_t.reshape(B, T, h_t.shape[0], K)) if inner == 1 else (q, q_t)
+    q = dueling_head(h, other, w, b, B, T, inner)
+    with th.no_grad() if frozen else th.enable_grad():
+        q_t = dueling_head(h_t, other, w_t, b_t, B, T, inner)
+    return q, q_t
 
 
 def _mix32p(x):
@@ -866,6 +926,108 @@
         return dx, dw, db, None
 
 
+def _bias_bmm_pair_fwd(x, w, b, x_t, w_t, b_t, leaky):
+    lib = abi.load_library()
+    x, w, b, x_t, w_t, b_t = (t.contiguous() for t in (x, w, b, x_t, w_t, b_t))
+    n, R, I = x.shape
+    n_t, O = x_t.shape[0], w.shape[2]
+    y = th.empty(n, R, O, dtype=th.float32, device=x.device)
+    y_t = th.empty(n_t, R, O, dtype=th.float32, device=x.device)
+    abi.check(lib, lib.ssd_bias_bmm_pair_fwd(x.data_ptr(), None, w.data_ptr(), b.data_ptr(), y.data_ptr(), n, x_t.data_ptr(), None, w_t.data_ptr(), b_t.data_ptr(),
+                                             y_t.data_ptr(), n_t, R, I, 0, O, 1, 0, int(bool(leaky)), _stream(x)))
+    return y, y_t
+
+
+class _BiasBmmPair(th.autograd.Function):
+
+    @staticmethod
+    def forward(ctx, x, w, b, leaky, x_t, w_t, b_t):
+        x, w = x.contiguous(), w.contiguous()
+        y, y_t = _bias_bmm_pair_fwd(x, w, b, x_t, w_t, b_t, leaky)
+        ctx.leaky = leaky
+        ctx.precision = LEARNER_PRECISION
+        ctx.save_for_backward(x, w, *((y,) if leaky else ()))
+        ctx.mark_non_differentiable(y_t)
+        ctx.set_materialize_grads(False)
+        return y, y_t
+
+    @staticmethod
+    def backward(ctx, g, g_t):
+        if g is None:
+            return (None,) * 7
+        with _precision(ctx.precision):
+            return _BiasBmm._backward(ctx, g) + (None, None, None)
+
+
+def bias_bmm_pair(x, w, b, x_t, w_t, b_t, leaky=False):
+    frozen = not (th.is_grad_enabled() and (x_t.requires_grad or w_t.requires_grad or b_t.requires_grad))
+    if (frozen and _bmm_kernel_ok(x, w, b) and _bmm_kernel_ok(x_t, w_t, b_t) and x_t.device == x.device and tuple(x_t.shape[1:]) == tuple(x.shape[1:])
+            and tuple(w_t.shape[1:]) == tuple(w.shape[1:])):
+        if th.is_grad_enabled() and (w.requires_grad or b.requires_grad or x.requires_grad):
+            return _BiasBmmPair.apply(x, w, b, leaky, x_t, w_t, b_t)
+        return _bias_bmm_pair_fwd(x, w, b, x_t, w_t, b_t, leaky)
+    y = bias_bmm(x, w, b, leaky)
+    with th.no_grad() if frozen else th.enable_grad():
+        y_t = bias_bmm(x_t, w_t, b_t, leaky)
+    return y, y_t
+
+
+class _Fc1Rows(th.autograd.Function):
+
+    @staticmethod
+    def forward(ctx, feat, tail, act, B, T, n, feat_t):
+        lib = abi.load_library()
+        feat, tail, act = feat.contiguous(), tail.contiguous(), act.contiguous()
+        F0, F1, A = feat.shape[1], tail.shape[1], act.shape[2]
+        new = lambda w: th.empty(n, T * B, w, dtype=th.float32, device=feat.device)
+        xe, xi = new(F0 + F1), new(F0 + F1 + A)
+        xe_t = xi_t = None
+        if feat_t is not None:
+            feat_t, xe_t, xi_t = feat_t.contiguous(), new(F0 + F1), new(F0 + F1 + A)
+        ptr = lambda t: None if t is None else t.data_ptr()
+        abi.check(lib, lib.ssd_fc1_rows_fwd(feat.data_ptr(), ptr(feat_t), tail.data_ptr(), act.data_ptr(), xe.data_ptr(), xi.data_ptr(), ptr(xe_t), ptr(xi_t),
+                                            B, T, n, F0, F1, A, _stream(feat)))
+        ctx.dims = (B, T, n, F0, F1, A)
+        ctx.set_materialize_grads(False)
+        if feat_t is None:
+            return xe, xi
+        ctx.mark_non_differentiable(xe_t, xi_t)
+        return xe, xi, xe_t, xi_t
+
+    @staticmethod
+    def backward(ctx, dxe, dxi, *unused):
+        lib = abi.load_library()
+        B, T, n, F0, F1, A = ctx.dims
+        if dxe is None and dxi is None:
+            return (None,) * 7
+        like = dxe if dxe is not None else dxi
+        dxe = like.new_zeros(n, T * B, F0 + F1) if dxe is None else dxe.contiguous()
+        dxi = like.new_zeros(n, T * B, F0 + F1 + A) if dxi is None else dxi.contiguous()
+        d_in = th.empty(B * T * n, F0 + F1, dtype=th.float32, device=dxe.device)
+        abi.check(lib, lib.ssd_fc1_rows_bwd(dxe.data_ptr(), dxi.data_ptr(), d_in.data_ptr(), B, T, n, F0, F1, A, F0 + F1, _stream(dxe)))
+        return d_in[:, :F0], None, None, None, None, None, None
+
+
+def fc1_rows(feat, tail, act, B, T, n, feat_t=None):
+    for name, t, shape in (("tail", tail, (B * T * n, tail.shape[-1])), ("act", act, (n, T * B, act.shape[-1]))) + (
+            () if feat_t is None else (("feat_t", feat_t, tuple(feat.shape)),)):
+        if tuple(t.shape) != shape or t.device != feat.device:
+            raise _unfit("fc1_rows", name, t, "%s on the device of feat expected" % (shape,))
+    if feat.dim() != 2 or feat.shape[0] != B * T * n:
+        raise _unfit("fc1_rows", "feat", feat, "[B * T * n = %d, F0] expected" % (B * T * n))
+    frozen = feat_t is None or not (th.is_grad_enabled() and feat_t.requires_grad)
+    if feat.is_cuda and frozen and _f32_on(feat, tail, act, *(() if feat_t is None else (feat_t,))) and tail.shape[1] >= 1 and not (
+            th.is_grad_enabled() and (tail.requires_grad or act.requires_grad)):
+        return _Fc1Rows.apply(feat, tail, act, B, T, n, feat_t)
+    _leaving_kernels("fc1_rows", feat, "dtypes / a tail or actions that ask for a gradient")
+    tm = lambda x: x.reshape(B, T, n, -1).permute(2, 1, 0, 3).reshape(n, T * B, -1)
+    out = ()
+    for f in (feat,) + (() if feat_t is None else (feat_t,)):
+        x = tm(th.cat([f, tail.to(f.dtype)], dim=1))
+        out += (x, th.cat([x, act.to(f.dtype)], dim=-1))
+    return out
+
+
 def bias_bmm(x, w, b, leaky=False):
     if _bmm_kernel_ok(x, w, b):
         if th.is_grad_enabled() and (w.requires_grad or b.requires_grad or x.requires_grad):
@@ -984,7 +1146,7 @@
         R = codes.shape[0]
         K = act[0].numel()
         st = _stream(codes)
-        g2 = th.ops.aten.leaky_relu_backward(d_feat.contiguous(), feat, 0.01, True)
+        g2 = th.ops.aten.leaky_relu_backward(d_feat, feat, 0.01, True).contiguous()
         d_lin_b = column_sums(g2)
         d_lin_w = th.empty(32, K, dtype=th.float32, device=codes.device)
         abi.check(lib, lib.ssd_bias_bmm_bwd(act.data_ptr(), g2.data_ptr(), None, None, d_lin_w.data_ptr(), None, None, 1, R, 32, K, st))
diff --git a/include/ssd_hip_train.h b/include/ssd_hip_train.h
--- /dev/null
+++ b/include/ssd_hip_train.h
@@ -0,0 +1,23 @@
+#ifndef SSD_HIP_TRAIN_H
+#define SSD_HIP_TRAIN_H
+
+#include "ssd_hip.h"
+
+#ifdef __cplusplus
+extern "C" {
+#endif
+
+int ssd_bias_bmm_pair_fwd(const float* x_a, const float* x2_a, const float* w_a, const float* b_a, float* y_a, int32_t n_a, const float* x_b,
+                          const float* x2_b, const float* w_b, const float* b_b, float* y_b, int32_t n_b, int32_t rows, int32_t in1, int32_t in2,
+                          int32_t out, int32_t x1_div, int32_t x2_shared, int32_t leaky, void* stream);
+int ssd_dueling_head_pair_fwd(const float* y_a, float* q_a, int32_t n_a, const float* y_b, float* q_b, int32_t n_b, int32_t T, int32_t B, int32_t inner,
+                              int32_t K, void* stream);
+int ssd_fc1_rows_fwd(const float* feat_a, const float* feat_b, const float* tail, const float* act, float* x_env_a, float* x_inc_a, float* x_env_b,
+                     float* x_inc_b, int32_t B, int32_t T, int32_t n, int32_t feat_w, int32_t tail_w, int32_t act_w, void* stream);
+int ssd_fc1_rows_bwd(const float* d_x_env, const float* d_x_inc, float* d_feat, int32_t B, int32_t T, int32_t n, int32_t feat_w, int32_t tail_w, int32_t act_w,
+                     int32_t d_feat_stride, void* stream);
+
+#ifdef __cplusplus
+}
+#endif
+#endif
```

Measured after the change: 351.4 million, median of 6. 1.0% higher.
